# wljungbergh/mpc-trajectory-generator

Hardware: AMD Instinct MI355X
Metric: nmpc_solves_per_sec (higher is better)
Workload: dtype f64

## Files before the change

### mpc_trajectory_generator_amd/csrc/nmpc_eval.h

```cpp
#pragma once

namespace nmpc {

struct WinState {
    int ctr;
    double xr, yr, mo2;
};
struct ObsCert {
    double xo, yo, m2;
    int act_lo, act_hi, act_dyn;
};
__device__ __forceinline__ int opaque_i(int x) { asm("" : "+v"(x)); return x; }
__device__ __forceinline__ bool window_is_global(double a2, double best, double mo2)
{
    const double t = mo2 - (a2 + best);
    return t > 1e-5 * mo2 && t * t > 4.0001 * (a2 * best);
}

__device__ __forceinline__ unsigned long long circle_near_mask(const double *p, int N, int nobs, int lane, double radius)
{
    const double *ps = p + NZ + N;
    bool keep = false;
    if (lane < nobs) {
        const double dx = ps[3 * lane] - p[0], dy = ps[3 * lane + 1] - p[1], r = ps[3 * lane + 2], lim = radius + r;
        keep = r > 0.0 && fma(dx, dx, dy * dy) <= lim * lim;
    }
    return __ballot(keep);
}

struct EvK { double ts, inv_ts, amin, amax, awmax; };
__device__ __forceinline__ double scalar_own(double x)
{
    int lo = __double2loint(x), hi = __double2hiint(x);
    asm volatile("" : "+v"(lo), "+v"(hi));
    return __hiloint2double(__builtin_amdgcn_readfirstlane(hi), __builtin_amdgcn_readfirstlane(lo));
}
__device__ __forceinline__ int scalar_own(int x)
{
    asm volatile("" : "+v"(x));
    return __builtin_amdgcn_readfirstlane(x);
}
struct EvX {
    double vprev, wprev;
    lds_double2 *mine;
    const lds_double2 *next;
};
template <int P, class SH = ShapeAny, bool WRITE_F2 = false, bool CULL = false, int WIN = 0, bool Z60 = false>
__device__ __forceinline__ void eval_psi(const KArgs &a, lds_double *L, int f2off, int lane, int t, double zv, double zw,
                                         double c, double cbar_inv, double yv, double yw, double vref, const DynStage &dyn,
                                         bool want_grad, double &psi, double &pen_out, double &gv,
                                         double &gw, double &av_out, double &aw_out, unsigned long long near = ~0ull, WinState *ws = nullptr,
                                         ObsCert *oc = nullptr, long long *nmpc_pe = nullptr, const EvK *ek = nullptr, const EvX *evx = nullptr)
{
    static_assert(!Z60 || P == 20, "zero pads in lanes 60..63: the tri layout only");
    const int N = shape_N<SH>(a), nobs = shape_nobs<SH>(a), ndyn = shape_ndyn<SH>(a);
    const LdsMap mp = the_map<SH, P>(a);
    const double ts = ek ? ek->ts : a.pb.ts, inv_ts = ek ? ek->inv_ts : a.inv_ts;
    const double k_amin = ek ? ek->amin : a.pb.amin, k_amax = ek ? ek->amax : a.pb.amax, k_awmax = ek ? ek->awmax : a.pb.awmax;
    (void)nmpc_pe;
    constexpr bool FULL = P == 20 && SH::N == 20;
    const bool in_r = t < N;
    const bool in = FULL ? true : in_r;
    const lds_double *sc = L + mp.sc;
    const double x0 = sc[SC_X0], y0 = sc[SC_Y0], th0 = sc[SC_TH0];
    const double xf = sc[SC_XF], yf = sc[SC_YF], thf = sc[SC_THF];

    double ew_, ex_, ey_;
    auto prefix_ex = [lane](double v, double &excl) {
        if constexpr (Z60) return group_prefix_ex_z60(v, lane, excl);
        else return group_prefix_ex<P>(v, lane, excl);
    };
    const double thn = fma(ts, prefix_ex(zw, ew_), th0);
    const double th = t == 0 ? th0 : fma(ts, ew_, th0);
    double sn, cs;
    sincos_cw_t(th, (const lds_double *)(L + mp.cw), sn, cs);
    const double xn = fma(ts, prefix_ex(zv * cs, ex_), x0);
    const double yn = fma(ts, prefix_ex(zv * sn, ey_), y0);
    const double xp = t == 0 ? x0 : fma(ts, ex_, x0);
    const double yp = t == 0 ? y0 : fma(ts, ey_, y0);

    const double half_c = 0.5 * c;
    NMPC_EVTICK(nmpc_pe, 0);

    double acc = (sc[SC_RV] * zv) * zv;
    acc = fma(sc[SC_RW] * zw, zw, acc);
    const double dv = zv - vref;
    acc = fma(sc[SC_QV] * dv, dv, acc);
    {
        const double ddx = xp - xf, ddy = yp - yf, dth = th - thf;
        acc = fma(sc[SC_Q], fma(ddx, ddx, ddy * ddy), acc);
        acc = fma(sc[SC_QTH] * dth, dth, acc);
    }
    double best = __builtin_inf();
    int bi = 0;
    bool full_scan = true;
    int i0c = 0;
    if constexpr (WIN > 0) {
        const int nseg = N - 1;
        if (nseg >= 2 * WIN + 1) {
            int cc = ws->ctr;
            cc = cc < 0 ? 0 : (cc > nseg - 1 ? nseg - 1 : cc);
            i0c = cc - WIN;
            i0c = i0c < 0 ? 0 : (i0c > nseg - (2 * WIN + 1) ? nseg - (2 * WIN + 1) : i0c);
            if (!__any(in_r & !(ws->mo2 > 0.0))) {
                const lds_double *sg = L + mp.seg + SEG_STRIDE * i0c;
                double wv[2 * WIN + 1][5];
#pragma unroll
                for (int j = 0; j <= 2 * WIN; ++j)
#pragma unroll
                    for (int f = 0; f < 5; ++f) wv[j][f] = sg[j * SEG_STRIDE + f];
#pragma unroll
                for (int j = 0; j <= 2 * WIN; ++j) {
                    const double px = xn - wv[j][0], py = yn - wv[j][1];
                    const double dot = fma(px, wv[j][2], py * wv[j][3]);
                    const double that = dot * wv[j][4];
                    const double tst = fmin(fmax(that, 0.0), 1.0);
                    const double ex = fma(tst, wv[j][2], -px), ey = fma(tst, wv[j][3], -py);
                    const double d2 = fma(ex, ex, ey * ey);
                    bi = d2 < best ? i0c + j : bi;
                    best = fmin(best, d2);
                }
                const double ax = xn - ws->xr, ay = yn - ws->yr;
                const bool sure = window_is_global(fma(ax, ax, ay * ay), best, ws->mo2);
                full_scan = __any(in_r & !sure);
                NMPC_WIN_COUNT(0, full_scan);
                if (full_scan) {
                    i0c = bi - WIN;
                    i0c = i0c < 0 ? 0 : (i0c > nseg - (2 * WIN + 1) ? nseg - (2 * WIN + 1) : i0c);
                    best = __builtin_inf(); bi = 0;
                }
            }
        }
    }
    if (full_scan) {
        const lds_double *sg = L + mp.seg;
        const int nseg4 = (N - 1 + 3) & ~3;
        double cur[2][5], nxt[2][5];
        double mout = __builtin_inf();
#pragma unroll
        for (int j = 0; j < 2; ++j)
#pragma unroll
            for (int f = 0; f < 5; ++f) cur[j][f] = sg[j * SEG_STRIDE + f];
#pragma unroll SH::N > 0 ? (SH::N <= 20 ? 32 : 2) : 1
        for (int i = 0; i < nseg4; i += 2) {
            sg += 2 * SEG_STRIDE;
#pragma unroll
            for (int j = 0; j < 2; ++j)
#pragma unroll
                for (int f = 0; f < 5; ++f) nxt[j][f] = sg[j * SEG_STRIDE + f];
            NMPC_SCHED_BARRIER();
            double d2[2];
#pragma unroll
            for (int j = 0; j < 2; ++j) {
                const double px = xn - cur[j][0], py = yn - cur[j][1];
                const double dot = fma(px, cur[j][2], py * cur[j][3]);
                const double that = dot * cur[j][4];
                const double tst = fmin(fmax(that, 0.0), 1.0);
                const double ex = fma(tst, cur[j][2], -px), ey = fma(tst, cur[j][3], -py);
                d2[j] = fma(ex, ex, ey * ey);
            }
#pragma unroll
            for (int j = 0; j < 2; ++j) {
                bi = d2[j] < best ? i + j : bi;
                best = fmin(best, d2[j]);
                if constexpr (WIN > 0) {
                    const int ie = i + j < N - 1 ? i + j : N - 2;
                    mout = (unsigned)(ie - i0c) <= 2u * WIN ? mout : fmin(mout, d2[j]);
                }
            }
            NMPC_SCHED_BARRIER();
#pragma unroll
            for (int j = 0; j < 2; ++j)
#pragma unroll
                for (int f = 0; f < 5; ++f) cur[j][f] = nxt[j][f];
        }
        if constexpr (WIN > 0) {
            const bool inw = (unsigned)(bi - i0c) <= 2u * WIN;
            ws->ctr = inw ? i0c + WIN : bi;
            ws->xr = xn; ws->yr = yn;
            ws->mo2 = inw && mout > 1e-8 ? mout : 0.0;
        }
    }
    NMPC_EVTICK(nmpc_pe, 1);
    acc = fma(sc[SC_QCTE], best, acc);
    const double vprev = evx ? evx->vprev : from_prev<P>(zv, lane, sc[SC_VINIT]);
    const double wprev = evx ? evx->wprev : from_prev<P>(zw, lane, sc[SC_WINIT]);
    double av = (zv - vprev) * inv_ts, aw = (zw - wprev) * inv_ts;
    acc = fma(sc[SC_PA] * av, av, acc);
    acc = fma(sc[SC_PW] * aw, aw, acc);
    const double tv = fma(yv, cbar_inv, av), tw = fma(yw, cbar_inv, aw);
    double sv = tv - clampd(tv, k_amin, k_amax);
    double sw = tw - clampd(tw, -k_awmax, k_awmax);
    acc = fma(half_c, fma(sv, sv, sw * sw), acc);
    if (t == N - 1) {
        const double tx = xn - xf, ty = yn - yf, tth = thn - thf;
        acc = fma(sc[SC_QN], fma(tx, tx, ty * ty), acc);
        acc = fma(sc[SC_QTHN] * tth, tth, acc);
    }
    if (!in) { acc = 0.0; av = aw = sv = sw = 0.0; }
    av_out = av;
    aw_out = aw;
    const double fsum = group_sum<P>(acc, lane);
    NMPC_EVTICK(nmpc_pe, 2);

    double pen = 0.0;
    unsigned long long act = 0ull;
    unsigned act_dyn = 0u;
    bool scan = true;
    if (oc) {
        const double ox = xn - oc->xo, oy = yn - oc->yo;
        const bool sure = fma(ox, ox, oy * oy) < oc->m2;
        if (!__any(in_r & !sure)) {
            act = ((unsigned long long)(unsigned)__builtin_amdgcn_readfirstlane(oc->act_hi) << 32) | (unsigned)__builtin_amdgcn_readfirstlane(oc->act_lo);
            act_dyn = (unsigned)__builtin_amdgcn_readfirstlane(oc->act_dyn);
            scan = false;
        }
        NMPC_WIN_COUNT(2, scan);
    }
    if (scan) {
        double mg = __builtin_inf();
        const lds_double *ob = L + mp.obs;
        const int nobs4 = (nobs + 3) & ~3;
        if constexpr (CULL) {
            const unsigned long long all = nobs >= 64 ? ~0ull : (1ull << nobs) - 1ull;
            unsigned long long todo = near & all;
            if (todo != all) {
                const double rx = xn - x0, ry = yn - y0;
                const double rg = 0.999 * a.cull_radius;
                const double ro2 = fma(rx, rx, ry * ry);
                if (__any(in_r & !(ro2 <= rg * rg))) todo = all;
                else if (oc) mg = rg - __builtin_amdgcn_sqrt(ro2);
            }
            while (todo) {
                int kk[4];
#pragma unroll
                for (int j = 0; j < 4; ++j) {
                    kk[j] = todo ? __builtin_ctzll(todo) : nobs;
                    todo &= todo - (todo ? 1ull : 0ull);
                }
                double od[16];
#pragma unroll
                for (int j = 0; j < 4; ++j) {
                    const lds_double *oj = ob + OBS_STRIDE * kk[j];
                    od[4 * j] = oj[0]; od[4 * j + 1] = oj[1]; od[4 * j + 2] = oj[2]; od[4 * j + 3] = oc ? oj[3] : 0.0;
                }
                NMPC_SCHED_BARRIER();
#pragma unroll
                for (int j = 0; j < 4; ++j) {
                    const double dx = xn - od[4 * j], dy = yn - od[4 * j + 1];
                    const double h = fma(-dy, dy, fma(-dx, dx, od[4 * j + 2]));
                    if (__any(in_r & (h > 0.0))) act |= 1ull << (kk[j] & 63);
                    else if (oc) mg = fmin(mg, __builtin_amdgcn_sqrt(od[4 * j + 2] - h) - od[4 * j + 3]);
                }
            }
        } else {
#pragma unroll SH::NOBS >= 0 && SH::NOBS <= 16 ? 16 : 1
        for (int k = 0; k < nobs4; k += 4, ob += 4 * OBS_STRIDE) {
            double od[16];
#pragma unroll
            for (int j = 0; j < 4; ++j) {
                od[4 * j] = ob[OBS_STRIDE * j]; od[4 * j + 1] = ob[OBS_STRIDE * j + 1]; od[4 * j + 2] = ob[OBS_STRIDE * j + 2];
                od[4 * j + 3] = oc ? ob[OBS_STRIDE * j + 3] : 0.0;
            }
            NMPC_SCHED_BARRIER();
#pragma unroll
            for (int j = 0; j < 4; ++j) {
                const double dx = xn - od[4 * j], dy = yn - od[4 * j + 1];
                const double h = fma(-dy, dy, fma(-dx, dx, od[4 * j + 2]));
                if (__any(in_r & (h > 0.0))) act |= 1ull << (k + j);
                else if (oc) mg = fmin(mg, __builtin_amdgcn_sqrt(od[4 * j + 2] - h) - od[4 * j + 3]);
            }
        }
        }
        NMPC_EVTICK(nmpc_pe, 5);
        {
            double dv_[NDYN_MAX][DY_FIELDS];
#pragma unroll
            for (int k = 0; k < NDYN_MAX; ++k)
#pragma unroll
                for (int f = 0; f < DY_FIELDS; ++f) dv_[k][f] = k < ndyn ? dyn.get(k, f) : 0.0;
            NMPC_SCHED_BARRIER();
#pragma unroll
            for (int k = 0; k < NDYN_MAX; ++k) {
                if (k < ndyn) {
                    const double ca = dv_[k][DY_CA], sa = dv_[k][DY_SA];
                    const double dx = xn - dv_[k][DY_EX], dy = yn - dv_[k][DY_EY];
                    const double ea = fma(dx, ca, dy * sa);
                    const double eb = fma(dx, sa, -(dy * ca));
                    const double h = fma(-(eb * eb), dv_[k][DY_IRY2], fma(-(ea * ea), dv_[k][DY_IRX2], 1.0));
                    if (__any(in_r & (h > 0.0))) act_dyn |= 1u << k;
                    else if (oc)
                        mg = fmin(mg, __builtin_amdgcn_sqrt(fma(dx, dx, dy * dy)) - __builtin_amdgcn_rsq(fmin(dv_[k][DY_IRX2], dv_[k][DY_IRY2])));
                }
            }
        }
        if (oc) {
            const double m = fma(0.99, mg, -1e-6);
            oc->xo = xn; oc->yo = yn;
            oc->m2 = m > 0.0 ? (m < 1e100 ? m * m : 1e200) : 0.0;
            oc->act_lo = opaque_i((int)(unsigned)act); oc->act_hi = opaque_i((int)(unsigned)(act >> 32)); oc->act_dyn = opaque_i((int)act_dyn);
        }
        NMPC_EVTICK(nmpc_pe, 6);
    }
    double gx = 0.0, gy = 0.0;
    if (want_grad) {
        const lds_double *sg = L + mp.seg + SEG_STRIDE * bi;
        const double px = xn - sg[0], py = yn - sg[1];
        const double dot = fma(px, sg[2], py * sg[3]);
        const double that = dot * sg[4];
        const double tst = fmin(fmax(that, 0.0), 1.0);
        const double ex = fma(tst, sg[2], -px), ey = fma(tst, sg[3], -py);
        const double ed = fma(ex, sg[2], ey * sg[3]);
        const double m = (that > 0.0 && that < 1.0) ? ed * sg[4] : 0.0;
        const double two_q = 2.0 * sc[SC_QCTE];
        gx = two_q * fma(m, sg[2], -ex);
        gy = two_q * fma(m, sg[3], -ey);
    }
    if ((act | act_dyn) != 0ull) {
        for (unsigned long long rem = act; rem;) {
            const int k0 = __builtin_ctzll(rem);
            rem &= rem - 1;
            if (rem == 0ull) {
                const lds_double *o0 = L + mp.obs + OBS_STRIDE * k0;
                const double ax = o0[0], ay = o0[1], ar = o0[2];
                const double dx0 = xn - ax, dy0 = yn - ay;
                const double h0 = fma(-dy0, dy0, fma(-dx0, dx0, ar));
                const double f20 = group_sum<P>(in ? fmax(h0, 0.0) : 0.0, lane);
                if (WRITE_F2 && t == 0) L[f2off + k0] = f20;
                pen = fma(f20, f20, pen);
                if (want_grad) {
                    const double w0 = -2.0 * (c * f20);
                    if (h0 > 0.0) { gx = fma(w0, dx0, gx); gy = fma(w0, dy0, gy); }
                }
                break;
            }
            const int k1 = __builtin_ctzll(rem);
            rem &= rem - 1;
            const lds_double *o0 = L + mp.obs + OBS_STRIDE * k0, *o1 = L + mp.obs + OBS_STRIDE * k1;
            const double ax = o0[0], ay = o0[1], ar = o0[2], bx = o1[0], by = o1[1], br = o1[2];
            const double dx0 = xn - ax, dy0 = yn - ay, dx1 = xn - bx, dy1 = yn - by;
            const double h0 = fma(-dy0, dy0, fma(-dx0, dx0, ar)), h1 = fma(-dy1, dy1, fma(-dx1, dx1, br));
            const double f20 = group_sum<P>(in ? fmax(h0, 0.0) : 0.0, lane);
            const double f21 = group_sum<P>(in ? fmax(h1, 0.0) : 0.0, lane);
            if (WRITE_F2 && t == 0) { L[f2off + k0] = f20; L[f2off + k1] = f21; }
            pen = fma(f20, f20, pen);
            pen = fma(f21, f21, pen);
            if (want_grad) {
                const double w0 = -2.0 * (c * f20), w1 = -2.0 * (c * f21);
                if (h0 > 0.0) { gx = fma(w0, dx0, gx); gy = fma(w0, dy0, gy); }
                if (h1 > 0.0) { gx = fma(w1, dx1, gx); gy = fma(w1, dy1, gy); }
            }
        }
#pragma unroll
        for (int k = 0; k < NDYN_MAX; ++k) {
            if (act_dyn & (1u << k)) {
                const double ca = dyn.get(k, DY_CA), sa = dyn.get(k, DY_SA);
                const double irx2 = dyn.get(k, DY_IRX2), iry2 = dyn.get(k, DY_IRY2);
                const double dx = xn - dyn.get(k, DY_EX), dy = yn - dyn.get(k, DY_EY);
                const double ea = fma(dx, ca, dy * sa);
                const double eb = fma(dx, sa, -(dy * ca));
                const double h = fma(-(eb * eb), iry2, fma(-(ea * ea), irx2, 1.0));
                const double f2 = group_sum<P>(in ? fmax(h, 0.0) : 0.0, lane);
                if (WRITE_F2 && t == 0) L[f2off + nobs + k] = f2;
                pen = fma(f2, f2, pen);
                if (want_grad) {
                    const double wk = -2.0 * (c * f2);
                    if (h > 0.0) {
                        const double A = ea * irx2, Bq = eb * iry2;
                        const double hx = fma(A, ca, Bq * sa);
                        const double hy = fma(A, sa, -(Bq * ca));
                        gx = fma(wk, hx, gx);
                        gy = fma(wk, hy, gy);
                    }
                }
            }
        }
    }
    psi = fma(half_c, pen, fsum);
    pen_out = pen;
    NMPC_EVTICK(nmpc_pe, 3);
    if (!want_grad) return;

    const double wq = t < N - 1 ? sc[SC_Q] : sc[SC_QN];
    const double wth = t < N - 1 ? sc[SC_QTH] : sc[SC_QTHN];
    gx = fma(2.0 * wq, xn - xf, gx);
    gy = fma(2.0 * wq, yn - yf, gy);
    double gt = (2.0 * wth) * (thn - thf);
    double qa = fma(c, sv, (2.0 * sc[SC_PA]) * av);
    double qw = fma(c, sw, (2.0 * sc[SC_PW]) * aw);
    if (!in) { gx = gy = gt = qa = qw = 0.0; }
    const double Sx = group_suffix<P>(gx, lane);
    const double Sy = group_suffix<P>(gy, lane);
    const double e = fma(Sy, cs, -(Sx * sn));
    const double Dt = in ? (ts * zv) * e : 0.0;
    const double St = group_suffix<P>(in ? gt + from_next<P>(Dt, lane) : 0.0, lane);
    double qan, qwn;
    if (evx) { *evx->mine = dbl2{qa, qw}; const dbl2 n_ = *evx->next; qan = n_.x; qwn = n_.y; }
    else { qan = from_next<P>(qa, lane); qwn = from_next<P>(qw, lane); }
    const double dynv = fma(Sx, cs, Sy * sn);
    double g1 = fma(2.0 * sc[SC_RV], zv, (2.0 * sc[SC_QV]) * dv);
    g1 = fma(inv_ts, qa - qan, g1);
    g1 = fma(ts, dynv, g1);
    double g2 = (2.0 * sc[SC_RW]) * zw;
    g2 = fma(inv_ts, qw - qwn, g2);
    g2 = fma(ts, St, g2);
    gv = in ? g1 : 0.0;
    gw = in ? g2 : 0.0;
    NMPC_EVTICK(nmpc_pe, 4);
}

template <int P>
__device__ __forceinline__ double hdot(double av, double aw, double bv, double bw, int lane)
{
    return group_sum<P>(fma(av, bv, aw * bw), lane);
}

template <int P>
__global__ __launch_bounds__(64) void nmpc_eval_kernel(KArgs a)
{
    extern __shared__ double lds[];
    constexpr int K = 64 / P;
    const int lane = threadIdx.x, g = lay_group<P>(lane), t = lay_stage<P>(lane);
    lds_double *L = (lds_double *)lds + g * a.map.total;
    const int N = a.pb.N;
    const bool in = t < N;
    const int inst = blockIdx.x * K + g;
    const int b = inst < a.B ? inst : a.B - 1;
    double vref;
    DynStage dyn;
    prepare_instance<P>(a, L, a.p + (size_t)b * a.n_p, t, vref, dyn);
    const double *u = a.u + (size_t)b * a.n_u;
    const double zv = in ? u[2 * t] : 0.0, zw = in ? u[2 * t + 1] : 0.0;
    const double c = a.ev_c ? a.ev_c[b] : 0.0;
    const double yv = (a.ev_y && in) ? a.ev_y[(size_t)b * a.n1 + t] : 0.0;
    const double yw = (a.ev_y && in) ? a.ev_y[(size_t)b * a.n1 + N + t] : 0.0;
    for (int k = t; k < a.n2; k += P) L[a.map.f2 + k] = 0.0;
    NMPC_WAVE_SYNC();
    double psi, pen, gv, gw, av, aw;
    eval_psi<P, ShapeAny, true>(a, L, a.map.f2, lane, t, zv, zw, c, 1.0 / fmax(c, 1.0), yv, yw, vref, dyn, true, psi, pen, gv, gw, av, aw);
    NMPC_WAVE_SYNC();
    if (inst >= a.B) return;
    if (t == 0 && a.ev_psi) a.ev_psi[b] = psi;
    if (in) {
        if (a.ev_grad) { a.ev_grad[(size_t)b * a.n_u + 2 * t] = gv; a.ev_grad[(size_t)b * a.n_u + 2 * t + 1] = gw; }
        if (a.ev_F1) { a.ev_F1[(size_t)b * a.n1 + t] = av; a.ev_F1[(size_t)b * a.n1 + N + t] = aw; }
    }
    if (a.ev_F2) for (int k = t; k < a.n2; k += P) a.ev_F2[(size_t)b * a.n2 + k] = L[a.map.f2 + k];
}

}
```

### mpc_trajectory_generator_amd/csrc/nmpc_layout.h

```cpp
#pragma once

#ifndef NMPC_WIN
#define NMPC_WIN 1
#endif

namespace nmpc {

constexpr int NZ = 20;
constexpr int MAXMEM = 10;
constexpr int NDYN_MAX = 3;
constexpr int GRAM_LD = 11;
constexpr int GRAM_NST = 20;
constexpr int OBS_STRIDE = 4;
constexpr int SEG_STRIDE = 5;
constexpr int TEAM_WAVES = 4;
constexpr int TEAM_REQ_DOUBLES = 3 * 24 * 2;
constexpr int TEAM_AREA_DOUBLES = 3 * 24 * 2 + 8;
constexpr int TEAM_CTL_INTS = 64;
constexpr int NPOOLS = 2;
enum { POOL_LONG = 0, POOL_COLD = 1 };

constexpr double GAMMA_L_COEFF = 0.95;
constexpr double DELTA_LIPSCHITZ = 1e-12;
constexpr double EPSILON_LIPSCHITZ = 1e-6;
constexpr double LIPSCHITZ_UPDATE_EPSILON = 1e-6;
constexpr int MAX_LIPSCHITZ_UPDATE_ITERATIONS = 10;
constexpr double MAX_LIPSCHITZ_CONSTANT = 1e9;
constexpr double MIN_LIPSCHITZ_CONSTANT = 1e-10;
constexpr int MAX_LINESEARCH_ITERATIONS = 10;
constexpr double LBFGS_SY_EPSILON = 1e-10;
constexpr double LBFGS_CBFGS_EPSILON = 1e-8;

struct LdsMap {
    int sc;
    int cw;
    int par;
    int seg;
    int obs;
    int f2;
    int dyn;
    int dyn_stride;
    int req;
    int vec;
    int rho;
    int S, Y;
    int nv;
    int gsy, gyy;
    int total;
};

struct KArgs {
    nmpc_problem pb;
    nmpc_opts op;
    LdsMap map;
    int B;
    int n_p, n_u, n1, n2;
    double inv_ts;
    const double *p;
    double *u;
    const double *y0;
    const double *c0;
    double *y_out;
    nmpc_status *st;
    unsigned int *queue;
    const int *order;
    int park_min;
    int park_depth;
    double *park;
    int *pool;
    unsigned int *pool_ctr;
    int pool_cap;
    int sched_mode;
    int sched_long_cap;
    int sched_cold_cap;
    int dbg;
    int team_owners;
    int team_help;
    double cull_radius;
    union {
        struct {
            const double *ev_c;
            const double *ev_y;
            double *ev_psi, *ev_grad, *ev_F1, *ev_F2;
        };
        struct {
            long long tl_dur;
            long long tl_budget;
            const long long *tl_t0;
        };
    };
};

enum { SC_X0 = 0, SC_Y0, SC_TH0, SC_VINIT, SC_WINIT, SC_XF, SC_YF, SC_THF,
       SC_Q, SC_QV, SC_QTH, SC_RV, SC_RW, SC_QN, SC_QTHN, SC_QCTE, SC_PA, SC_PW };

typedef __attribute__((address_space(3))) double lds_double;
typedef double dbl2 __attribute__((ext_vector_type(2)));
typedef __attribute__((address_space(3))) dbl2 lds_double2;

#ifdef NMPC_NO_SCHED_BARRIER
#define NMPC_SCHED_BARRIER() do { } while (0)
#else
#define NMPC_SCHED_BARRIER() __builtin_amdgcn_sched_barrier(0)
#endif
#define NMPC_WAVE_SYNC()                                           \
    do {                                                           \
        __builtin_amdgcn_fence(__ATOMIC_RELEASE, "workgroup");     \
        __builtin_amdgcn_wave_barrier();                           \
        __builtin_amdgcn_fence(__ATOMIC_ACQUIRE, "workgroup");     \
    } while (0)

enum { DY_EX = 0, DY_EY, DY_CA, DY_SA, DY_IRX2, DY_IRY2, DY_FIELDS };
struct DynStage {
    const lds_double *col;
    int stride;
    __device__ __forceinline__ double get(int k, int f) const { return col[(k * DY_FIELDS + f) * stride]; }
};

struct ShapeAny { static constexpr int N = 0, NOBS = -1, NDYN = -1; };
struct ShapeDefault { static constexpr int N = 20, NOBS = 10, NDYN = 3; };
struct ShapeNobs50 { static constexpr int N = 20, NOBS = 50, NDYN = 3; };
struct ShapeN40 { static constexpr int N = 40, NOBS = 10, NDYN = 3; };
template <class S> struct Timed { static constexpr int N = S::N, NOBS = S::NOBS, NDYN = S::NDYN; };
template <class SH> struct ShapeTimed { static constexpr bool value = false; };
template <class S> struct ShapeTimed<Timed<S>> { static constexpr bool value = true; };
template <class SH> __device__ __forceinline__ int shape_N(const KArgs &a) { if constexpr (SH::N > 0) return SH::N; else return a.pb.N; }
template <class SH> __device__ __forceinline__ int shape_nobs(const KArgs &a) { if constexpr (SH::NOBS >= 0) return SH::NOBS; else return a.pb.nobs; }
template <class SH> __device__ __forceinline__ int shape_ndyn(const KArgs &a) { if constexpr (SH::NDYN >= 0) return SH::NDYN; else return a.pb.ndyn; }

__host__ __device__ constexpr LdsMap lds_layout(int N, int nobs, int ndyn, int P)
{
    LdsMap mp{};
    int o = 0;
    mp.sc = o;  o += 20;
    mp.cw = o;  o += CW_NCOEF;
    mp.par = o; o += 24;
    mp.seg = o; o += SEG_STRIDE * (N + 5);
    mp.obs = o; o += OBS_STRIDE * (nobs + 4);
    const int points = P == 64 ? 1 : 3;
    mp.f2 = o;  o += P == 20 ? 0 : points * (nobs + ndyn + 1);
    mp.rho = o; o += MAXMEM;
    const int cols = P == 20 ? 24 : P;
    mp.dyn_stride = P == 64 ? ((N + 1) & ~1) : (P == 20 ? 24 : P);
    mp.dyn = o; o += NDYN_MAX * 6 * mp.dyn_stride;
    o = (o + 1) & ~1;
    mp.req = o; o += P == 20 ? TEAM_REQ_DOUBLES : 0;
    mp.vec = o; o += P == 64 ? 0 : 7 * 2 * cols;
    if (P == 20) { mp.f2 = mp.vec; if (7 * 2 * cols < points * (nobs + ndyn + 1)) o = mp.vec + points * (nobs + ndyn + 1); }
    o = (o + 1) & ~1;
    mp.gsy = o; o += P == 20 ? MAXMEM * GRAM_LD : 0;
    mp.gyy = o; o += P == 20 ? MAXMEM * GRAM_LD : 0;
    const int ring = P == 20 ? GRAM_NST + 1 : N;
    mp.S = o;   o += 2 * ring * MAXMEM;
    mp.Y = o;   o += 2 * ring * MAXMEM;
    mp.nv = o;  o += P == 20 ? 4 * 2 * GRAM_NST : 0;
    mp.total = (o + 1) & ~1;
    if (P == 20 && mp.total < 3 * TEAM_WAVES * TEAM_AREA_DOUBLES) mp.total = 3 * TEAM_WAVES * TEAM_AREA_DOUBLES;
    return mp;
}
template <class SH, int P> __device__ __forceinline__ LdsMap the_map(const KArgs &a)
{
    if constexpr (SH::N > 0 && SH::NOBS >= 0 && SH::NDYN >= 0) return lds_layout(SH::N, SH::NOBS, SH::NDYN, P);
    else return a.map;
}

template <int P, class SH = ShapeAny>
__device__ __forceinline__ void prepare_instance(const KArgs &a, lds_double *L, const double *p, int t,
                                                 double &vref, DynStage &dyn)
{
    const int N = shape_N<SH>(a), nobs = shape_nobs<SH>(a), ndyn = shape_ndyn<SH>(a);
    const LdsMap mp = the_map<SH, P>(a);
    if (t < 8) L[mp.sc + t] = p[t];
    if (t >= 8 && t < 18) L[mp.sc + t] = p[t + 2];
    if (t == 18 || t == 19) L[mp.sc + t] = p[t - 15];
    if (t < CW_NCOEF) L[mp.cw + t] = CW_COEF_DEV[t];
    NMPC_WAVE_SYNC();
    vref = t < N ? p[NZ + t] : 0.0;
    const double *ps = p + NZ + N;
    for (int k = t; k < ((nobs + 4) & ~3); k += P) {
        const bool real = k < nobs;
        const double r = real ? ps[3 * k + 2] : 0.0;
        L[mp.obs + OBS_STRIDE * k] = real ? ps[3 * k] : 0.0;
        L[mp.obs + OBS_STRIDE * k + 1] = real ? ps[3 * k + 1] : 0.0;
        L[mp.obs + OBS_STRIDE * k + 2] = r * r;
        L[mp.obs + OBS_STRIDE * k + 3] = r > 0.0 ? r : -1e30;
    }
    const double *pd = ps + 3 * nobs;
    {
        lds_double *col = L + mp.dyn + t;
        dyn.col = col;
        const int ds = P == 64 ? mp.dyn_stride : lay_cols<P>();
        dyn.stride = ds;
#pragma unroll
        for (int k = 0; k < NDYN_MAX; ++k) {
            double ex = 0.0, ey = 0.0, ca = 0.0, sa = 0.0, irx2 = 1.0, iry2 = 1.0;
            if (k < ndyn && t < N) {
                const double *e = pd + (k * N + t) * 5;
                ex = e[0];
                ey = e[1];
                irx2 = 1.0 / (e[2] * e[2]);
                iry2 = 1.0 / (e[3] * e[3]);
                sincos_cw_t(e[4], (const lds_double *)(L + mp.cw), sa, ca);
            }
            if (P != 64 || t < ds) {
                col[(k * DY_FIELDS + DY_EX) * ds] = ex;
                col[(k * DY_FIELDS + DY_EY) * ds] = ey;
                col[(k * DY_FIELDS + DY_CA) * ds] = ca;
                col[(k * DY_FIELDS + DY_SA) * ds] = sa;
                col[(k * DY_FIELDS + DY_IRX2) * ds] = irx2;
                col[(k * DY_FIELDS + DY_IRY2) * ds] = iry2;
            }
        }
    }
    const double *pr = pd + 5 * ndyn * N;
    const int nseg4 = (N - 1 + 3) & ~3;
    if (t < nseg4) {
        const int i = t < N - 1 ? t : N - 2;
        const double ax = pr[3 * i], ay = pr[3 * i + 1];
        const double bx = pr[3 * i + 3], by = pr[3 * i + 4];
        const double dx = bx - ax, dy = by - ay;
        lds_double *sg = L + mp.seg + SEG_STRIDE * t;
        sg[0] = ax;
        sg[1] = ay;
        sg[2] = dx;
        sg[3] = dy;
        sg[4] = 1.0 / (fma(dx, dx, dy * dy) + 1e-16);
    }
    NMPC_WAVE_SYNC();
}

__host__ __device__ inline int park_stride(int N) { return 6 * N + 16; }
}
```

### mpc_trajectory_generator_amd/csrc/nmpc_solve_hyb.h

```cpp
#pragma once

#ifndef NMPC_CULL_MIN
#define NMPC_CULL_MIN 16
#endif
#ifndef NMPC_WIN
#define NMPC_WIN 1
#endif

namespace nmpc {

typedef __attribute__((address_space(3))) int lds_int;
enum { CTL_OWNERS = 0, CTL_HELPERS = 1, CTL_CLAIM = 4, CTL_DONE = 8, CTL_INST = 56 };
__device__ __forceinline__ int ctl_load(lds_int *p) { return __hip_atomic_load(p, __ATOMIC_RELAXED, __HIP_MEMORY_SCOPE_WORKGROUP); }
__device__ __forceinline__ void ctl_store(lds_int *p, int v) { __hip_atomic_store(p, v, __ATOMIC_RELAXED, __HIP_MEMORY_SCOPE_WORKGROUP); }
__device__ __forceinline__ int ctl_add(lds_int *p, int v) { return __hip_atomic_fetch_add(p, v, __ATOMIC_RELAXED, __HIP_MEMORY_SCOPE_WORKGROUP); }

__device__ __forceinline__ double point_scalar(double v, int k)
{
    const int lo = __builtin_amdgcn_readlane(__double2loint(v), 16 * k);
    const int hi = __builtin_amdgcn_readlane(__double2hiint(v), 16 * k);
    return __hiloint2double(hi, lo);
}

#define NMPC_FETCH_GRAD(K, OV, OW)                                             \
    do {                                                                       \
        const dbl2 fg_ = zgr[(K) * ZS];                                        \
        OV = fg_.x; OW = fg_.y;                                                \
    } while (0)

#define NMPC_HALF_STEP(xv, xw)                                                 \
    do {                                                                       \
        const double s1_ = fma(-gamma, gv, (xv)), s2_ = fma(-gamma, gw, (xw)); \
        hv = ina ? clampd(s1_, vmin, vmax) : s1_;                              \
        hw = ina ? clampd(s2_, -wmax, wmax) : s2_;                             \
    } while (0)
#define NMPC_FBE(xv, xw) fbe_value<P>(cost, gamma, pk_hig, fma(-gamma, gv, (xv)), fma(-gamma, gw, (xw)), hv, hw, gv, gw, lane)

constexpr int POOL_CTRS = 4;
__device__ __forceinline__ int pool_pop(const KArgs &a, int c)
{
    unsigned int *ctr = a.pool_ctr + POOL_CTRS * c;
    int *cnt = (int *)(ctr + 2);
    if (__hip_atomic_load(cnt, __ATOMIC_RELAXED, __HIP_MEMORY_SCOPE_AGENT) <= 0) return -1;
    if (__hip_atomic_fetch_add(cnt, -1, __ATOMIC_RELAXED, __HIP_MEMORY_SCOPE_AGENT) <= 0) {
        __hip_atomic_fetch_add(cnt, 1, __ATOMIC_RELAXED, __HIP_MEMORY_SCOPE_AGENT);
        return -1;
    }
    const unsigned pos = __hip_atomic_fetch_add(&ctr[0], 1u, __ATOMIC_RELAXED, __HIP_MEMORY_SCOPE_AGENT);
    int *slot = a.pool + (size_t)c * a.pool_cap + pos % (unsigned)a.pool_cap;
    int inst;
    do { inst = __hip_atomic_load(slot, __ATOMIC_ACQUIRE, __HIP_MEMORY_SCOPE_AGENT); } while (inst < 0);
    __hip_atomic_store(slot, -1, __ATOMIC_RELAXED, __HIP_MEMORY_SCOPE_AGENT);
    return inst;
}
__device__ __forceinline__ void pool_push(const KArgs &a, int c, int inst)
{
    unsigned int *ctr = a.pool_ctr + POOL_CTRS * c;
    const unsigned pos = __hip_atomic_fetch_add(&ctr[1], 1u, __ATOMIC_RELAXED, __HIP_MEMORY_SCOPE_AGENT);
    int *slot = a.pool + (size_t)c * a.pool_cap + pos % (unsigned)a.pool_cap;
    while (__hip_atomic_load(slot, __ATOMIC_RELAXED, __HIP_MEMORY_SCOPE_AGENT) >= 0) __builtin_amdgcn_s_sleep(1);
    __hip_atomic_store(slot, inst, __ATOMIC_RELEASE, __HIP_MEMORY_SCOPE_AGENT);
    __hip_atomic_fetch_add((int *)(ctr + 2), 1, __ATOMIC_RELEASE, __HIP_MEMORY_SCOPE_AGENT);
}
__device__ __forceinline__ int pool_depth(const KArgs &a, int c)
{
    return __hip_atomic_load((int *)(a.pool_ctr + POOL_CTRS * c + 2), __ATOMIC_RELAXED, __HIP_MEMORY_SCOPE_AGENT);
}

template <int J>
__device__ __forceinline__ double fnma_row_bcast(double acc, double x, double y)
{
    asm("s_nop 1\n\tv_fmac_f64_dpp %0, -%1, %2 row_newbcast:%3 row_mask:0xf bank_mask:0xf" : "+v"(acc) : "v"(x), "v"(y), "n"(J));
    return acc;
}
template <int J>
__device__ __forceinline__ double fma_row_bcast(double acc, double x, double y)
{
    asm("s_nop 1\n\tv_fmac_f64_dpp %0, %1, %2 row_newbcast:%3 row_mask:0xf bank_mask:0xf" : "+v"(acc) : "v"(x), "v"(y), "n"(J));
    return acc;
}
template <int J>
__device__ __forceinline__ void fnma3_row_bcast(double &a1, double &a2, double &a3, double x, double y1, double y2, double y3, double after)
{
    asm("v_fmac_f64_dpp %0, -%3, %4 row_newbcast:%8 row_mask:0xf bank_mask:0xf\n\t"
        "v_fmac_f64_dpp %1, -%3, %5 row_newbcast:%8 row_mask:0xf bank_mask:0xf\n\t"
        "v_fmac_f64_dpp %2, -%3, %6 row_newbcast:%8 row_mask:0xf bank_mask:0xf"
        : "+v"(a1), "+v"(a2), "+v"(a3) : "v"(x), "v"(y1), "v"(y2), "v"(y3), "v"(after), "n"(J));
}
template <int J>
__device__ __forceinline__ void fma2_row_bcast(double &a1, double &a2, double x, double y1, double y2, double after)
{
    asm("v_fmac_f64_dpp %0, %2, %3 row_newbcast:%6 row_mask:0xf bank_mask:0xf\n\t"
        "v_fmac_f64_dpp %1, %2, %4 row_newbcast:%6 row_mask:0xf bank_mask:0xf"
        : "+v"(a1), "+v"(a2) : "v"(x), "v"(y1), "v"(y2), "v"(after), "n"(J));
}
template <int J>
__device__ __forceinline__ void fnma2_row_bcast(double &a1, double &a2, double x, double y1, double y2, double after)
{
    asm("v_fmac_f64_dpp %0, -%2, %3 row_newbcast:%6 row_mask:0xf bank_mask:0xf\n\t"
        "v_fmac_f64_dpp %1, -%2, %4 row_newbcast:%6 row_mask:0xf bank_mask:0xf"
        : "+v"(a1), "+v"(a2) : "v"(x), "v"(y1), "v"(y2), "v"(after), "n"(J));
}
template <int J>
__device__ __forceinline__ void fnma5_row_bcast(double &a1, double &a2, double &a3, double &a4, double &a5, double x, double y1, double y2, double y3,
                                                double y4, double y5, double after)
{
    asm("v_fmac_f64_dpp %0, -%5, %6 row_newbcast:%12 row_mask:0xf bank_mask:0xf\n\t"
        "v_fmac_f64_dpp %1, -%5, %7 row_newbcast:%12 row_mask:0xf bank_mask:0xf\n\t"
        "v_fmac_f64_dpp %2, -%5, %8 row_newbcast:%12 row_mask:0xf bank_mask:0xf\n\t"
        "v_fmac_f64_dpp %3, -%5, %9 row_newbcast:%12 row_mask:0xf bank_mask:0xf\n\t"
        "v_fmac_f64_dpp %4, -%5, %10 row_newbcast:%12 row_mask:0xf bank_mask:0xf"
        : "+v"(a1), "+v"(a2), "+v"(a3), "+v"(a4), "+v"(a5) : "v"(x), "v"(y1), "v"(y2), "v"(y3), "v"(y4), "v"(y5), "v"(after), "n"(J));
}
template <int J>
__device__ __forceinline__ void fma4_row_bcast(double &a1, double &a2, double &a3, double &a4, double x, double y1, double y2, double y3, double y4,
                                               double after)
{
    asm("v_fmac_f64_dpp %0, %4, %5 row_newbcast:%10 row_mask:0xf bank_mask:0xf\n\t"
        "v_fmac_f64_dpp %1, %4, %6 row_newbcast:%10 row_mask:0xf bank_mask:0xf\n\t"
        "v_fmac_f64_dpp %2, %4, %7 row_newbcast:%10 row_mask:0xf bank_mask:0xf\n\t"
        "v_fmac_f64_dpp %3, %4, %8 row_newbcast:%10 row_mask:0xf bank_mask:0xf"
        : "+v"(a1), "+v"(a2), "+v"(a3), "+v"(a4) : "v"(x), "v"(y1), "v"(y2), "v"(y3), "v"(y4), "v"(after), "n"(J));
}
__device__ __forceinline__ double lane_scalar(double v, int ln)
{
    const int lo = __builtin_amdgcn_readlane(__double2loint(v), ln);
    const int hi = __builtin_amdgcn_readlane(__double2hiint(v), ln);
    return __hiloint2double(hi, lo);
}
template <int J>
__device__ __forceinline__ double gram_fwd_step(double &ga1, double &ga2, double &dv, double &dw, double rho, double gs, double gy, double alp,
                                                double ypx, double ypy)
{
    double al;
    asm("v_mul_f64 %0, %5, %1\n\t"
        "v_fmac_f64_dpp %3, -%8, %9 row_newbcast:%12 row_mask:0xf bank_mask:0xf\n\t"
        "v_fmac_f64_dpp %4, -%8, %10 row_newbcast:%12 row_mask:0xf bank_mask:0xf\n\t"
        "v_fmac_f64_dpp %1, -%0, %6 row_newbcast:%11 row_mask:0xf bank_mask:0xf\n\t"
        "v_fmac_f64_dpp %2, -%0, %7 row_newbcast:%11 row_mask:0xf bank_mask:0xf"
        : "=&v"(al), "+v"(ga1), "+v"(ga2), "+v"(dv), "+v"(dw)
        : "v"(rho), "v"(gs), "v"(gy), "v"(alp), "v"(ypx), "v"(ypy), "n"(J), "n"(J - 1));
    return al;
}
__device__ __forceinline__ double gram_fwd_first(double &ga1, double &ga2, double rho, double gs, double gy)
{
    double al;
    asm("v_mul_f64 %0, %3, %1\n\t"
        "s_nop 1\n\t"
        "v_fmac_f64_dpp %1, -%0, %4 row_newbcast:0 row_mask:0xf bank_mask:0xf\n\t"
        "v_fmac_f64_dpp %2, -%0, %5 row_newbcast:0 row_mask:0xf bank_mask:0xf"
        : "=&v"(al), "+v"(ga1), "+v"(ga2) : "v"(rho), "v"(gs), "v"(gy));
    return al;
}
template <int J>
__device__ __forceinline__ double gram_bwd_step(double &ga2, double &dv, double &dw, double rho, double alv, double gr, double abp, double spx,
                                                double spy)
{
    double ab;
    asm("v_mul_f64 %0, %4, %1\n\t"
        "v_add_f64 %0, %5, -%0\n\t"
        "v_fmac_f64_dpp %2, %7, %8 row_newbcast:%11 row_mask:0xf bank_mask:0xf\n\t"
        "v_fmac_f64_dpp %3, %7, %9 row_newbcast:%11 row_mask:0xf bank_mask:0xf\n\t"
        "v_fmac_f64_dpp %1, %0, %6 row_newbcast:%10 row_mask:0xf bank_mask:0xf"
        : "=&v"(ab), "+v"(ga2), "+v"(dv), "+v"(dw)
        : "v"(rho), "v"(alv), "v"(gr), "v"(abp), "v"(spx), "v"(spy), "n"(J), "n"(J + 1));
    return ab;
}
#define NMPC_GRAM_LDF(H, J)                                                                    \
        constexpr int fp##J = ((H) + (J)) % MAXMEM;                                            \
        const double fgs##J = Lgsy[pkrow + fp##J], fgy##J = Lgyy[pkrow + fp##J];               \
        const dbl2 fyp##J = LY[fp##J * NS + tt]
#define NMPC_GRAM_FWD(H, J, JP)                                                                \
        NMPC_GRAM_LDF(H, J);                                                                   \
        const double fal##J = gram_fwd_step<(J)>(ga1, ga2, dv, dw, rho_k, fgs##J, fgy##J, fal##JP, fyp##JP.x, fyp##JP.y)
#define NMPC_GRAM_LDB(H, J)                                                                    \
        constexpr int bp##J = ((H) + (J)) % MAXMEM;                                            \
        const double bgr##J = Lgsy[bp##J * GRAM_LD + pk_];                                     \
        const dbl2 bsp##J = LS[bp##J * NS + tt]
#define NMPC_GRAM_BWD(H, J, JP)                                                                \
        NMPC_GRAM_LDB(H, J);                                                                   \
        const double bab##J = gram_bwd_step<(J)>(ga2, dv, dw, rho_k, alv, bgr##J, bab##JP, bsp##JP.x, bsp##JP.y)
#define NMPC_GRAM_BOTH(H)                                                                                                            \
    do {                                                                                                                             \
        NMPC_GRAM_LDF(H, 0);                                                                                                         \
        const double fal0 = gram_fwd_first(ga1, ga2, rho_k, fgs0, fgy0);                                                             \
        NMPC_GRAM_FWD(H, 1, 0); NMPC_GRAM_FWD(H, 2, 1); NMPC_GRAM_FWD(H, 3, 2); NMPC_GRAM_FWD(H, 4, 3); NMPC_GRAM_FWD(H, 5, 4);      \
        NMPC_GRAM_FWD(H, 6, 5); NMPC_GRAM_FWD(H, 7, 6); NMPC_GRAM_FWD(H, 8, 7); NMPC_GRAM_FWD(H, 9, 8);                              \
        fnma2_row_bcast<9>(dv, dw, fal9, fyp9.x, fyp9.y, ga1);                                                                      \
        const double alv = rho_k * ga1;                        \
        ga2 = n_H0 * ga2;                                                                                                            \
        dv = n_H0 * dv; dw = n_H0 * dw;                                                                                              \
        NMPC_GRAM_LDB(H, 9);                                                                                                         \
        const double bab9 = alv - rho_k * ga2;                                                                                       \
        ga2 = fma_row_bcast<9>(ga2, bab9, bgr9);                                                                                     \
        NMPC_GRAM_BWD(H, 8, 9); NMPC_GRAM_BWD(H, 7, 8); NMPC_GRAM_BWD(H, 6, 7); NMPC_GRAM_BWD(H, 5, 6); NMPC_GRAM_BWD(H, 4, 5);      \
        NMPC_GRAM_BWD(H, 3, 4); NMPC_GRAM_BWD(H, 2, 3); NMPC_GRAM_BWD(H, 1, 2); NMPC_GRAM_BWD(H, 0, 1);                              \
        fma2_row_bcast<0>(dv, dw, bab0, bsp0.x, bsp0.y, ga2);                                                                        \
    } while (0)

struct FlagBit {
    unsigned &w;
    const unsigned bit;
    __device__ __forceinline__ operator bool() const { return (w & bit) != 0u; }
    __device__ __forceinline__ FlagBit &operator=(bool v) { w = v ? (w | bit) : (w & ~bit); return *this; }
    __device__ __forceinline__ FlagBit &operator=(const FlagBit &o) { return *this = (bool)o; }
};

template <class SH>
__global__ __launch_bounds__(64 * TEAM_WAVES, 2) void nmpc_solve_hyb_kernel(KArgs a)
{
    static_assert(MAXMEM == 10, "the Gram-form recurrences are written out for ten pairs");
    constexpr int PE = 20;
    constexpr int P = 32, COLS = 24;
    extern __shared__ double lds[];
    const int wid = __builtin_amdgcn_readfirstlane((int)(threadIdx.x >> 6));
    const int slice = the_map<SH, PE>(a).total;
    lds_double *L = (lds_double *)lds + wid * slice;
    lds_int *ctl = (lds_int *)((lds_double *)lds + TEAM_WAVES * slice);
    const int lane = threadIdx.x & 63, h = lane >> 5, t = lane & 31;
    const int q = lay_group<PE>(lane), te = lay_stage<PE>(lane);
    const int N = shape_N<SH>(a), m = scalar_own(a.op.lbfgs_memory);
    const int k_akkt = scalar_own(a.op.akkt_gradient), k_lsf = scalar_own(a.op.ls_failure);
#ifdef NMPC_EXPERIMENTS
    const int k_help = scalar_own(a.team_help), k_dbg = scalar_own(a.dbg);
#else
    constexpr int k_help = 1, k_dbg = 0;
#endif
    const bool in = t < N, ina = in;
    const bool ine = te < N;
    constexpr bool FULL = SH::N == PE;
    constexpr bool CULL = SH::NOBS > NMPC_CULL_MIN || SH::NOBS < 0;
    constexpr int WIN = NMPC_WIN;
    constexpr bool OBSC = SH::N > 0;
    const bool inea = FULL ? true : ine;
    const LdsMap mp = the_map<SH, PE>(a);
    const int n2 = shape_nobs<SH>(a) + shape_ndyn<SH>(a);
    const int f2off = mp.f2 + q * (n2 + 1);
    constexpr int ZS = 24, src0 = 0, src1 = 1, src2 = 2;
    static_assert(3 * ZS + 8 == 4 * GRAM_NST, "the transport area is the place of the Gram batch's four vectors");
    lds_double2 *Lz = (lds_double2 *)(L + mp.nv);
    lds_double2 *zwX = Lz + (t < ZS ? h * ZS + t : 3 * ZS + (t - ZS));
    lds_double2 *zwY = Lz + (t < ZS ? 2 * ZS + t : 3 * ZS + (t - ZS));
    const lds_double2 *zrd = Lz + q * ZS + te;
    const lds_double2 *zpv = te == 0 ? (const lds_double2 *)(L + mp.sc + 18) : (lane < 60 ? zrd - 1 : zrd);
    lds_double2 *zmine = Lz + (lane < 60 ? q * ZS + te : 3 * ZS + (lane - 60));
    const lds_double2 *znext = Lz + opaque_i(lane < 60 ? q * ZS + te + 1 : 3 * ZS + (lane - 60) + 1);
    const lds_double2 *zgr = Lz + (t < 20 ? t : 20);
    constexpr int NS = GRAM_NST + 1;
    const int tt = t < GRAM_NST ? t : GRAM_NST;
    lds_double2 *LS = (lds_double2 *)(L + mp.S);
    lds_double2 *LY = (lds_double2 *)(L + mp.Y);
    lds_double *Lrho = L + mp.rho;
    lds_double2 *Lnv = (lds_double2 *)(L + mp.nv);
    lds_double *Lgsy = L + mp.gsy, *Lgyy = L + mp.gyy;
    const int c16 = lane & 15, q4 = lane >> 4;
    lds_double2 *Los = (lds_double2 *)(L + mp.vec) + (t < COLS ? t : COLS - 1);
    lds_double2 *Log = Los + COLS, *Lq = Los + 2 * COLS, *Lyp = Los + 3 * COLS;
    lds_double2 *Lgk = Los + 6 * COLS;
    lds_double2 *LypE = (lds_double2 *)(L + mp.vec) + 3 * COLS + te;
    lds_double2 *Ly = (lds_double2 *)(L + mp.vec) + 4 * COLS + te;
    lds_double *Lvr = L + mp.vec + 2 * 5 * COLS + te;
#define NMPC_LB_ZERO()                                                                                  \
    do {                                                                                                \
        lds_double2 *z_ = (lds_double2 *)(L + mp.gsy);                                                  \
        for (int i_ = lane; i_ < MAXMEM * GRAM_LD + 2 * MAXMEM * NS; i_ += 64) z_[i_] = dbl2{0.0, 0.0};  \
        if (lane < MAXMEM) Lrho[lane] = 0.0;                                                            \
    } while (0)
    if (threadIdx.x < TEAM_CTL_INTS) ctl[threadIdx.x] = threadIdx.x == CTL_OWNERS ? a.team_owners : 0;
    __syncthreads();
    lds_double2 *Lreq = (lds_double2 *)(L + mp.req);
    unsigned team_seq = 0;
    const double vmin = scalar_own(a.pb.vmin), vmax = scalar_own(a.pb.vmax), wmax = scalar_own(a.pb.wmax);
    const EvK ek = {scalar_own(a.pb.ts), scalar_own(a.inv_ts), scalar_own(a.pb.amin), scalar_own(a.pb.amax), scalar_own(a.pb.awmax)};
    const double tol_ = scalar_own(a.op.tolerance);
    const unsigned max_inner = (unsigned)scalar_own(a.op.max_inner);
    const unsigned budget = (unsigned)scalar_own(a.op.max_total_inner);
    constexpr bool TIMED = ShapeTimed<SH>::value;
    long long clk_batch = CLK_NEVER, clk_dl = CLK_NEVER;
    if constexpr (TIMED) { if (a.tl_budget > 0) clk_batch = uniform_ll(*a.tl_t0) + a.tl_budget; }
    lds_double *Lpar = L + mp.par;
#define pk_eps_nu Lpar[0]
#define pk_dy_norm Lpar[1]
#define pk_f2_norm Lpar[2]
#define pk_dy_norm_plus Lpar[3]
#define pk_f2_norm_plus Lpar[4]
#define pk_last_fpr Lpar[5]
#define pk_last_cost Lpar[6]
#define pk_norm_h Lpar[7]
#define pk_Lc Lpar[8]
#define pk_H0 Lpar[9]
#define pk_sigma Lpar[10]
#define pk_c_lip Lpar[11]
#define pk_fbe_u Lpar[20]
#define pk_hig Lpar[19]
#define pk_gr Lpar[12]


    const unsigned hw_slot = __builtin_amdgcn_s_getreg(((4 - 1) << 11) | (0 << 6) | 4);
    const bool unfavoured = hw_slot != 0u;
    const int PS = park_stride(N);

    const int n_waves = (int)gridDim.x * TEAM_WAVES;
    if (a.order && unfavoured && a.park_min > 0 && a.B >= n_waves + (n_waves >> 2)) {
        const unsigned want = (unsigned)n_waves / 2;
        const long long t_hold = (long long)__builtin_amdgcn_s_memrealtime();
        while (__hip_atomic_load(a.queue, __ATOMIC_RELAXED, __HIP_MEMORY_SCOPE_AGENT) < want &&
               (long long)__builtin_amdgcn_s_memrealtime() - t_hold < 4000)
            __builtin_amdgcn_s_sleep(8);
    }

    for (; wid < a.team_owners;) {
        int fetched = -1, from_pool = 0;
        if (lane == 0) {
            const bool pools = a.park_min > 0 || a.sched_mode > 0;
            if (pools && !unfavoured) { fetched = pool_pop(a, POOL_LONG); from_pool = fetched >= 0; }
            if (fetched < 0) {
                const unsigned nxt = atomicAdd(a.queue, 1u);
                if (nxt < (unsigned)a.B) fetched = a.order ? a.order[nxt] : (int)nxt;
                else if (pools) {
                    for (int c = 0; c < NPOOLS && fetched < 0; ++c) fetched = pool_pop(a, c);
                    from_pool = fetched >= 0;
                }
            }
        }
        const int inst = __builtin_amdgcn_readfirstlane(fetched);
        const bool resumed = __builtin_amdgcn_readfirstlane(from_pool) != 0;
        if (inst < 0) break;

        const long long dbg_t0 = __builtin_amdgcn_s_memtime();
        const auto clk0_ = __builtin_amdgcn_s_memrealtime();
        long long t_first = (long long)clk0_;
        Lpar[13] = (double)clk0_; Lpar[14] = 0.0;
        if (k_dbg == 1) { if (hw_slot & 1u) __builtin_amdgcn_s_setprio(0); else __builtin_amdgcn_s_setprio(3); }
        double vref_;
        DynStage dyn;
        if (lane == 0) ctl_store(ctl + CTL_INST + wid, -1);
        __builtin_amdgcn_fence(__ATOMIC_RELEASE, "workgroup");
        prepare_instance<PE, SH>(a, L, a.p + (size_t)inst * a.n_p, te, vref_, dyn);
        *Lvr = vref_;
        WinState ws = {te < N - 1 ? te : N - 2, 0.0, 0.0, 0.0};
        ObsCert oc = {0.0, 0.0, 0.0, 0, 0, 0};
        __builtin_amdgcn_fence(__ATOMIC_RELEASE, "workgroup");
        if (lane == 0) ctl_store(ctl + CTL_INST + wid, inst);
        unsigned long long near = ~0ull;
        if constexpr (CULL) {
            near = circle_near_mask(a.p + (size_t)inst * a.n_p, N, shape_nobs<SH>(a), lane, a.cull_radius);
            if (lane == 0) { Lpar[18] = __hiloint2double((int)(near >> 32), (int)near); }
        }

        const double *pk = a.park + (size_t)inst * PS;
        const double *u0 = resumed ? pk : a.u + (size_t)inst * a.n_u;
        double uv = in ? u0[2 * t] : 0.0, uw = in ? u0[2 * t + 1] : 0.0;
        {
            double yv0, yw0;
            if (resumed) {
                yv0 = ine ? pk[2 * N + 2 * te] : 0.0;
                yw0 = ine ? pk[2 * N + 2 * te + 1] : 0.0;
            } else {
                yv0 = (a.y0 && ine) ? a.y0[(size_t)inst * a.n1 + te] : 0.0;
                yw0 = (a.y0 && ine) ? a.y0[(size_t)inst * a.n1 + N + te] : 0.0;
            }
            *LypE = dbl2{yv0, yw0};
            *Ly = dbl2{yv0, yw0};
        }
        *Lq = (resumed && in) ? dbl2{pk[4 * N + 2 * t], pk[4 * N + 2 * t + 1]} : dbl2{0.0, 0.0};
        double gv = 0, gw = 0, hv = 0, hw = 0, rv = 0, rw = 0, dv = 0, dw = 0;
        unsigned fl = 0u;
        FlagBit need_grad{fl, 1u << 0}; need_grad = true;
        double cost = 0, gamma = 0, tau = 1, rhs_ls = 0;
        pk_fbe_u = 0.0; pk_hig = 0.0;
        pk_Lc = 0.0; pk_sigma = 0.0; pk_H0 = 1.0;
        FlagBit fbe_ok{fl, 1u << 1};
        int iteration = 0, lip_it = 0, ls_n = 0, lb_active = 0, lb_head = 0;
        FlagBit lb_first{fl, 1u << 2}; lb_first = true;
        int n_active = 0, n_head = 0;
        FlagBit n_first{fl, 1u << 3}, n_take_old{fl, 1u << 4}; n_first = true;
        double n_H0 = 1;
        unsigned num_iter = 0;
        const double c0 = a.c0 ? a.c0[inst] : 0.0;
        double pen_c = c0 > 0.0 ? c0 : a.op.initial_penalty;
        double cbar_inv = 1.0 / fmax(pen_c, 1.0);
        pk_c_lip = 0.0;
        pk_eps_nu = a.op.initial_tolerance;
        pk_dy_norm = 0.0; pk_f2_norm = 0.0; pk_dy_norm_plus = DBL_MAX; pk_f2_norm_plus = 0.0; pk_last_fpr = 0.0; pk_last_cost = 0.0; pk_norm_h = 0.0;
        int nu = 0, inner_status = 0, state = D_INIT, final_status = 0;
        unsigned inner_total = 0, n_cost = 0, n_grad = 0, n_pass = 0;
        FlagBit parked{fl, 1u << 5};
        int park_cls = POOL_LONG;
        unsigned q_pass = 0;
        FlagBit long_counted{fl, 1u << 6};
        if (resumed) {
            const double *pks = a.park + (size_t)inst * PS + 6 * N;
            pen_c = pks[0];
            cbar_inv = 1.0 / fmax(pen_c, 1.0);
            pk_eps_nu = pks[1]; pk_dy_norm = pks[2]; pk_f2_norm = pks[3]; pk_dy_norm_plus = pks[4]; pk_f2_norm_plus = pks[5];
            pk_last_fpr = pks[6]; pk_last_cost = pks[7];
            nu = (int)pks[8]; inner_total = (unsigned)pks[9]; n_cost = (unsigned)pks[10]; n_grad = (unsigned)pks[11]; n_pass = (unsigned)pks[12];
            Lpar[13] = pks[13]; Lpar[14] = pks[14] + 1.0;
            if constexpr (TIMED) t_first = (long long)pks[13];
            long_counted = pks[15] != 0.0; q_pass = n_pass;
        }
        if constexpr (TIMED) clk_dl = clk_deadline(clk_batch, a.tl_dur, t_first);

        FlagBit f_start{fl, 1u << 7}, f_back{fl, 1u << 8}, f_trials{fl, 1u << 9}, f_begin{fl, 1u << 11}, f_done{fl, 1u << 12}, f_fb{fl, 1u << 13};
        FlagBit running{fl, 1u << 14}, timed_out{fl, 1u << 15};
        f_start = true; running = true;
        FlagBit posted{fl, 1u << 16};
        FlagBit clk_late{fl, 1u << 17};
        NMPC_PROBE_STATE

#define NMPC_END_ITERATION()                                                                                   \
        do {                                                                                                   \
            iteration++;                                                                                       \
            if (!(num_iter < max_inner)) f_done = true;                                                        \
            else {                                                                                             \
                num_iter++;                                                                                    \
                if ((budget > 0u && inner_total + num_iter >= budget) || (TIMED && clk_late)) { timed_out = true; f_done = true; } \
                else f_begin = true;                                                                           \
            }                                                                                                  \
        } while (0)
        for (;;) {
            double xv = 0, xw = 0, yqv = 0, yqw = 0;
            double nr2 = 0, norm_r = 0;
            double pv = 0, pw = 0;
            bool lb_batch = false;
            if (fl & (f_back.bit | f_fb.bit)) {
                if (f_back) {
                    if (posted) { posted = false; if (lane == 0) ctl_store(ctl + CTL_CLAIM + wid, 0); }
                    lb_active = 0; lb_first = true;
                    NMPC_LB_ZERO();
                    fbe_ok = false;
                    pk_Lc *= 2.0; gamma /= 2.0;
                    pk_sigma = (1.0 - GAMMA_L_COEFF) / (4.0 * gamma);
                    pk_c_lip = GAMMA_L_COEFF / (2.0 * gamma);
                    pk_hig = 0.5 / gamma;
                    NMPC_HALF_STEP(uv, uw);
                    lb_batch = true;
                }
                if (f_fb) {
                    f_fb = false;
                    tau = 0.0;
                    { const dbl2 gk_ = *Lgk; gv = gk_.x; gw = gk_.y; }
                    NMPC_HALF_STEP(uv, uw);
                    xv = yqv = hv; xw = yqw = hw; need_grad = true; state = D_FB;
                }
            }
            if (f_trials) {
                f_trials = false;
                const double th_ = h == 0 ? tau : tau / 2.0, omt = 1.0 - th_;
                xv = fma(-th_, dv, fma(-omt, rv, uv));
                xw = fma(-th_, dw, fma(-omt, rw, uw));
                const double t4_ = tau / 4.0, om4_ = 1.0 - t4_;
                yqv = fma(-t4_, dv, fma(-om4_, rv, uv));
                yqw = fma(-t4_, dw, fma(-om4_, rw, uw));
                need_grad = true; state = D_LS;
            }
            if (f_begin) lb_batch = true;
            if (f_begin) { NMPC_TL_STEP(); NMPC_TL_EV(tl_it, 0); }
            NMPC_SEC(0);
            double gU = 0.0, gs1 = 0.0, gs2 = 0.0, gy1 = 0.0, gy2 = 0.0;
            if (lb_batch) {
                rv = uv - hv; rw = uw - hw;
                if (f_begin && iteration >= 1 && !lb_first) {
                    const dbl2 os_ = *Los, og_ = *Log;
                    gs1 = uv - os_.x; gs2 = uw - os_.y; gy1 = rv - og_.x; gy2 = rw - og_.y;
                }
                if (t < GRAM_NST && h == 0) {
                    Lnv[t] = dbl2{gs1, gs2}; Lnv[GRAM_NST + t] = dbl2{gy1, gy2};
                    Lnv[2 * GRAM_NST + t] = dbl2{rv, rw}; Lnv[3 * GRAM_NST + t] = dbl2{gv, gw};
                }
                const lds_double2 *X1 = (c16 < MAXMEM ? LS + c16 * NS : (c16 == 11 ? Lnv + 2 * GRAM_NST : Lnv)) + 5 * q4;
                const lds_double2 *X2 = (c16 < MAXMEM ? LY + c16 * NS : (c16 == 11 ? Lnv + 3 * GRAM_NST : Lnv + GRAM_NST)) + 5 * q4;
                const lds_double2 *Z1 = (c16 < MAXMEM ? Lnv + GRAM_NST : (c16 == 10 ? Lnv : Lnv + 2 * GRAM_NST)) + 5 * q4;
                const lds_double2 *Z2 = (c16 < MAXMEM ? Lnv + 2 * GRAM_NST : (c16 == 10 ? Lnv + GRAM_NST : Lnv + 2 * GRAM_NST)) + 5 * q4;
                double V1 = 0.0, V2 = 0.0, V3 = 0.0, V4 = 0.0;
#pragma unroll
                for (int e = 0; e < 5; ++e) {
                    const dbl2 x1 = X1[e], x2 = X2[e], z1 = Z1[e], z2 = Z2[e];
                    V1 = fma(x1.x, z1.x, V1); V1 = fma(x1.y, z1.y, V1);
                    V2 = fma(x1.x, z2.x, V2); V2 = fma(x1.y, z2.y, V2);
                    V3 = fma(x2.x, z1.x, V3); V3 = fma(x2.y, z1.y, V3);
                    V4 = fma(x2.x, z2.x, V4); V4 = fma(x2.y, z2.y, V4);
                }
                swap_rows(V1, V2);
                const double W12 = V1 + V2;
                swap_rows(V3, V4);
                double W34 = V3 + V4;
                double W12b = W12;
                swap_halves(W12b, W34);
                gU = W12b + W34;
                nr2 = lane_scalar(gU, 11);
                pk_gr = lane_scalar(gU, 32 + 11);
                norm_r = sqrt(nr2);
                pk_last_fpr = norm_r;
                NMPC_SEC_KEEP(norm_r + gU);
            }
            NMPC_SEC(1);
            if (lb_batch) { NMPC_TL_KEEP(norm_r + gU); NMPC_TL_EV(tl_it, 1); }
            if (f_begin) {
                f_begin = false;
                bool exit_now = false;
                if (__any(norm_r < tol_)) {
                    if (k_akkt == 2) exit_now = true;
                    else if (k_akkt == 1 && iteration >= 1) {
                        exit_now = __any(norm_r < pk_eps_nu * gamma);
                    } else {
                        const dbl2 q_ = *Lq;
                        const bool top = k_akkt == 1;
                        const double b1 = top ? gv : gv - q_.x;
                        const double b2 = top ? gw : gw - q_.y;
                        const double a1 = rv / gamma + b1, a2 = rw / gamma + b2;
                        exit_now = __any(sqrt(group_sum<P>(fma(a1, a1, a2 * a2), lane)) < pk_eps_nu);
                    }
                }
                if (exit_now) {
                    f_done = true;
                } else if (iteration == 0) {
                    lip_it = 0;
                    xv = yqv = hv; xw = yqw = hw; need_grad = true; state = D_LIP;
                } else {
                    lip_it = 0;
                    n_first = lb_first; n_head = lb_head; n_active = lb_active; n_H0 = pk_H0; n_take_old = false;
                    bool took = false;
                    if (lb_first) {
                        n_first = false; n_take_old = true;
                    } else {
                        const double ss = lane_scalar(gU, 10), ys = lane_scalar(gU, 16 + 10);
                        bool ok = !(ss <= DBL_MIN || ys <= LBFGS_SY_EPSILON);
                        if (ok) ok = ys > (LBFGS_CBFGS_EPSILON * norm_r) * ss;
                        if (__any(ok)) {
                            took = true;
                            n_take_old = true;
                            n_head = lb_head == 0 ? MAXMEM - 1 : lb_head - 1;
                            if (in && h == 0) { LS[n_head * NS + t] = dbl2{gs1, gs2}; LY[n_head * NS + t] = dbl2{gy1, gy2}; }
                            if (lane == 0) Lrho[n_head] = 1.0 / ys;
                            const double yy = lane_scalar(gU, 48 + 10);
                            n_H0 = ys / yy;
                            if (n_active < m) n_active++;
                            if (c16 < MAXMEM && q4 < 3) {
                                const bool dg = c16 == n_head;
                                lds_double *wa = q4 == 0 ? Lgsy + c16 * GRAM_LD + n_head : (q4 == 1 ? Lgsy + n_head * GRAM_LD + c16 : Lgyy + c16 * GRAM_LD + n_head);
                                const double wv = q4 == 1 ? 0.0 : (dg ? (q4 == 0 ? 0.0 : yy) : gU);
                                *wa = wv;
                                if (q4 == 2) Lgyy[n_head * GRAM_LD + c16] = wv;
                            }
                            if (m < MAXMEM) {
                                const int ev = n_head + m >= MAXMEM ? n_head + m - MAXMEM : n_head + m;
// ... 492 lines not shown
```

### mpc_trajectory_generator_amd/csrc/nmpc_solve_hyb2.h

```cpp
#pragma once

namespace nmpc {

struct D2 { double a, b; };
__device__ __forceinline__ D2 d2s(double s) { return D2{s, s}; }
__device__ __forceinline__ D2 operator+(D2 x, D2 y) { return D2{x.a + y.a, x.b + y.b}; }
__device__ __forceinline__ D2 operator-(D2 x, D2 y) { return D2{x.a - y.a, x.b - y.b}; }
__device__ __forceinline__ D2 operator*(D2 x, D2 y) { return D2{x.a * y.a, x.b * y.b}; }
__device__ __forceinline__ D2 operator*(double s, D2 y) { return D2{s * y.a, s * y.b}; }
__device__ __forceinline__ D2 operator-(D2 x) { return D2{-x.a, -x.b}; }
__device__ __forceinline__ D2 fma2(D2 x, D2 y, D2 z) { return D2{fma(x.a, y.a, z.a), fma(x.b, y.b, z.b)}; }
__device__ __forceinline__ D2 fma2(double s, D2 y, D2 z) { return D2{fma(s, y.a, z.a), fma(s, y.b, z.b)}; }
__device__ __forceinline__ D2 fma2(double s, D2 y, double z) { return D2{fma(s, y.a, z), fma(s, y.b, z)}; }
__device__ __forceinline__ D2 sel2(bool ca, bool cb, D2 x, D2 y) { return D2{ca ? x.a : y.a, cb ? x.b : y.b}; }
__device__ __forceinline__ D2 clamp2(D2 x, double lo, double hi) { return D2{clampd(x.a, lo, hi), clampd(x.b, lo, hi)}; }

__device__ __forceinline__ double gsum2(D2 v, int lane) { return group_sum<20>(v.a + v.b, lane); }
__device__ __forceinline__ D2 gprefix2(D2 v, int lane)
{
    double E;
    const double W = group_prefix_ex<20>(v.a + v.b, lane, E);
    return D2{E + v.a, W};
}
__device__ __forceinline__ D2 gsuffix2(D2 v, int lane)
{
    const double Z = group_suffix<20>(v.a + v.b, lane);
    return D2{Z, from_next<20>(Z, lane) + v.b};
}
__device__ __forceinline__ D2 prev2(D2 v, int lane, double fill) { return D2{from_prev<20>(v.b, lane, fill), v.a}; }
__device__ __forceinline__ D2 next2(D2 v, int lane) { return D2{v.b, from_next<20>(v.a, lane)}; }

__device__ __forceinline__ double hdot2(D2 av, D2 aw, D2 bv, D2 bw) { return fma(av.a, bv.a, aw.a * bw.a) + fma(av.b, bv.b, aw.b * bw.b); }

template <int CNT> __device__ __forceinline__ void ld4(const lds_double2 *blk, int e, D2 &v, D2 &w)
{
    const dbl2 c0 = blk[e], c1 = blk[CNT + e];
    v = D2{c0.x, c1.x};
    w = D2{c0.y, c1.y};
}
template <int CNT> __device__ __forceinline__ void st4(lds_double2 *blk, int e, D2 v, D2 w)
{
    blk[e] = dbl2{v.a, w.a};
    blk[CNT + e] = dbl2{v.b, w.b};
}

struct LdsMap2 {
    int sc, cw, par, seg, obs, f2, rho;
    int dyn;
    int vr;
    int pts;
    int grd;
    int req;
    int vec;
    int gsy, gyy;
    int S, Y;
    int nv;
    int total;
};
#ifndef NMPC_WIN2
#define NMPC_WIN2 1
#endif
constexpr int H2_COLS = 24, H2_NS = 21, H2_ENT = 24;
constexpr int TEAM2_AREA_DOUBLES = 3 * H2_ENT * 4 + 8;
__host__ __device__ constexpr LdsMap2 lds_layout2(int N, int nobs, int ndyn)
{
    LdsMap2 mp{};
    int o = 0;
    mp.sc = o;  o += 20;
    mp.cw = o;  o += CW_NCOEF;
    mp.par = o; o += 20;
    mp.seg = o; o += SEG_STRIDE * (N + 5);
    mp.obs = o; o += OBS_STRIDE * (nobs + 4);
    mp.f2 = o;  o += 0;
    mp.rho = o; o += MAXMEM;
    o = (o + 1) & ~1;
    mp.dyn = o; o += NDYN_MAX * 6 * 48;
    mp.vr = o;  o += 48;
    mp.pts = o; o += 3 * H2_ENT * 4;
    mp.grd = o; o += 3 * H2_ENT * 4;
    mp.req = o; o += 3 * H2_ENT * 4;
    mp.vec = o; o += 7 * H2_COLS * 4;
    mp.f2 = mp.vec;
    if (7 * H2_COLS * 4 < 3 * (nobs + ndyn + 1)) o = mp.vec + 3 * (nobs + ndyn + 1);
    o = (o + 1) & ~1;
    mp.gsy = o; o += MAXMEM * GRAM_LD;
    mp.gyy = o; o += MAXMEM * GRAM_LD;
    mp.S = o;   o += MAXMEM * H2_NS * 4;
    mp.Y = o;   o += MAXMEM * H2_NS * 4;
    mp.nv = mp.pts;
    mp.total = (o + 1) & ~1;
    return mp;
}
template <class SH> __device__ __forceinline__ LdsMap2 the_map2(const KArgs &a)
{
    if constexpr (SH::N > 0 && SH::NOBS >= 0 && SH::NDYN >= 0) return lds_layout2(SH::N, SH::NOBS, SH::NDYN);
    else return lds_layout2(a.pb.N, a.pb.nobs, a.pb.ndyn);
}

template <class SH>
__device__ __forceinline__ void prepare_instance2(const KArgs &a, lds_double *L, const LdsMap2 &mp, const double *p, int lane)
{
    const int N = shape_N<SH>(a), nobs = shape_nobs<SH>(a), ndyn = shape_ndyn<SH>(a);
    if (lane < 8) L[mp.sc + lane] = p[lane];
    if (lane >= 8 && lane < 18) L[mp.sc + lane] = p[lane + 2];
    if (lane < CW_NCOEF) L[mp.cw + lane] = CW_COEF_DEV[lane];
    NMPC_WAVE_SYNC();
    if (lane < 48) L[mp.vr + lane] = lane < N ? p[NZ + lane] : 0.0;
    const double *ps = p + NZ + N;
    for (int k = lane; k < ((nobs + 3) & ~3); k += 64) {
        const bool real = k < nobs;
        const double r = real ? ps[3 * k + 2] : 0.0;
        L[mp.obs + OBS_STRIDE * k] = real ? ps[3 * k] : 0.0;
        L[mp.obs + OBS_STRIDE * k + 1] = real ? ps[3 * k + 1] : 0.0;
        L[mp.obs + OBS_STRIDE * k + 2] = r * r;
        L[mp.obs + OBS_STRIDE * k + 3] = r > 0.0 ? r : -1e30;
    }
    const double *pd = ps + 3 * nobs;
    if (lane < 48) {
        lds_double *col = L + mp.dyn + lane;
#pragma unroll
        for (int k = 0; k < NDYN_MAX; ++k) {
            double ex = 0.0, ey = 0.0, ca = 0.0, sa = 0.0, irx2 = 1.0, iry2 = 1.0;
            if (k < ndyn && lane < N) {
                const double *e = pd + (k * N + lane) * 5;
                ex = e[0];
                ey = e[1];
                irx2 = 1.0 / (e[2] * e[2]);
                iry2 = 1.0 / (e[3] * e[3]);
                sincos_cw_t(e[4], (const lds_double *)(L + mp.cw), sa, ca);
            }
            col[(k * DY_FIELDS + DY_EX) * 48] = ex;
            col[(k * DY_FIELDS + DY_EY) * 48] = ey;
            col[(k * DY_FIELDS + DY_CA) * 48] = ca;
            col[(k * DY_FIELDS + DY_SA) * 48] = sa;
            col[(k * DY_FIELDS + DY_IRX2) * 48] = irx2;
            col[(k * DY_FIELDS + DY_IRY2) * 48] = iry2;
        }
    }
    const double *pr = pd + 5 * ndyn * N;
    const int nseg4 = (N - 1 + 3) & ~3;
    if (lane < nseg4) {
        const int i = lane < N - 1 ? lane : N - 2;
        const double ax = pr[3 * i], ay = pr[3 * i + 1];
        const double bx = pr[3 * i + 3], by = pr[3 * i + 4];
        const double dx = bx - ax, dy = by - ay;
        lds_double *sg = L + mp.seg + SEG_STRIDE * lane;
        sg[0] = ax;
        sg[1] = ay;
        sg[2] = dx;
        sg[3] = dy;
        sg[4] = 1.0 / (fma(dx, dx, dy * dy) + 1e-16);
    }
    NMPC_WAVE_SYNC();
}

__device__ __forceinline__ D2 dyn2(const lds_double *L, const LdsMap2 &mp, int te, int k, int f)
{
    const dbl2 v = ((const lds_double2 *)(L + mp.dyn + (k * DY_FIELDS + f) * 48))[te];
    return D2{v.x, v.y};
}

struct ObsCert2 {
    D2 xo, yo, m2;
    int act_lo, act_hi, act_dyn;
};
template <class SH, bool WRITE_F2 = false, int WIN = 0>
__device__ __forceinline__ void eval_psi2(const KArgs &a, lds_double *L, const LdsMap2 &mp, int f2off, int lane, int te, D2 zv, D2 zw,
                                          double c, double cbar_inv, D2 yv, D2 yw, bool want_grad, double &psi, double &pen_out,
                                          D2 &gv, D2 &gw, D2 &av_out, D2 &aw_out, WinState *ws = nullptr, ObsCert2 *oc = nullptr)
{
    const int N = shape_N<SH>(a), nobs = shape_nobs<SH>(a), ndyn = shape_ndyn<SH>(a);
    const double ts = a.pb.ts, inv_ts = a.inv_ts;
    constexpr bool FULL = SH::N == 40;
    const int sa_ = 2 * te, sb_ = 2 * te + 1;
    const bool ra = sa_ < N, rb = sb_ < N;
    const bool ina = FULL ? true : ra, inb = FULL ? true : rb;
    const lds_double *sc = L + mp.sc;
    const lds_double *cw = (const lds_double *)(L + mp.cw);
    const double x0 = sc[SC_X0], y0 = sc[SC_Y0], th0 = sc[SC_TH0];
    const double xf = sc[SC_XF], yf = sc[SC_YF], thf = sc[SC_THF];
    D2 vref;
    { const dbl2 v = ((const lds_double2 *)(L + mp.vr))[te]; vref = D2{v.x, v.y}; }

    const D2 thn = fma2(ts, gprefix2(zw, lane), th0);
    const D2 th = prev2(thn, lane, th0);
    D2 sn, cs;
    sincos_cw_t(th.a, cw, sn.a, cs.a);
    sincos_cw_t(th.b, cw, sn.b, cs.b);
    const D2 xn = fma2(ts, gprefix2(zv * cs, lane), x0);
    const D2 yn = fma2(ts, gprefix2(zv * sn, lane), y0);
    const D2 xp = prev2(xn, lane, x0);
    const D2 yp = prev2(yn, lane, y0);
    const double half_c = 0.5 * c;

    D2 acc = (sc[SC_RV] * zv) * zv;
    acc = fma2(sc[SC_RW] * zw, zw, acc);
    const D2 dv = zv - vref;
    acc = fma2(sc[SC_QV] * dv, dv, acc);
    {
        const D2 ddx = xp - d2s(xf), ddy = yp - d2s(yf), dth = th - d2s(thf);
        acc = fma2(sc[SC_Q], fma2(ddx, ddx, ddy * ddy), acc);
        acc = fma2(sc[SC_QTH] * dth, dth, acc);
    }
    const D2 vprev = prev2(zv, lane, sc[SC_VINIT]);
    const D2 wprev = prev2(zw, lane, sc[SC_WINIT]);
    D2 best = d2s(__builtin_inf());
    int bia = 0, bib = 0;
    bool full_scan = true;
    int i0a = 0, i0b = 0;
    if constexpr (WIN > 0) {
        const int nseg = N - 1;
        if (nseg >= 2 * WIN + 1) {
#define NMPC2_CLAMP_WIN(C_) ((C_) - WIN < 0 ? 0 : ((C_) - WIN > nseg - (2 * WIN + 1) ? nseg - (2 * WIN + 1) : (C_) - WIN))
            { const int ca = ws[0].ctr < 0 ? 0 : (ws[0].ctr > nseg - 1 ? nseg - 1 : ws[0].ctr); i0a = NMPC2_CLAMP_WIN(ca); }
            { const int cb = ws[1].ctr < 0 ? 0 : (ws[1].ctr > nseg - 1 ? nseg - 1 : ws[1].ctr); i0b = NMPC2_CLAMP_WIN(cb); }
            if (!__any((ra & !(ws[0].mo2 > 0.0)) | (rb & !(ws[1].mo2 > 0.0)))) {
                bool sure_a, sure_b;
#define NMPC2_WINDOW(S_, BI_, I0_, WS_, SURE_)                                                             \
                do {                                                                                       \
                    const lds_double *sg = L + mp.seg + SEG_STRIDE * (I0_);                                \
                    double bst = __builtin_inf();                                                          \
                    int bi_ = 0;                                                                           \
                    _Pragma("unroll") for (int j = 0; j <= 2 * WIN; ++j) {                                 \
                        const double s0 = sg[j * SEG_STRIDE], s1 = sg[j * SEG_STRIDE + 1], s2 = sg[j * SEG_STRIDE + 2], \
                                     s3 = sg[j * SEG_STRIDE + 3], s4 = sg[j * SEG_STRIDE + 4];             \
                        const double px = xn.S_ - s0, py = yn.S_ - s1;                                     \
                        const double dot = fma(s2, px, s3 * py);                                           \
                        const double tst = fmin(fmax(s4 * dot, 0.0), 1.0);                                 \
                        const double ex = fma(s2, tst, -px), ey = fma(s3, tst, -py);                       \
                        const double d2 = fma(ex, ex, ey * ey);                                            \
                        bi_ = d2 < bst ? (I0_) + j : bi_;                                                  \
                        bst = fmin(bst, d2);                                                               \
                    }                                                                                      \
                    const double ax = xn.S_ - (WS_).xr, ay = yn.S_ - (WS_).yr;                             \
                    SURE_ = window_is_global(fma(ax, ax, ay * ay), bst, (WS_).mo2);                        \
                    best.S_ = bst; BI_ = bi_;                                                              \
                } while (0)
                NMPC2_WINDOW(a, bia, i0a, ws[0], sure_a);
                NMPC2_WINDOW(b, bib, i0b, ws[1], sure_b);
#undef NMPC2_WINDOW
                full_scan = __any((ra & !sure_a) | (rb & !sure_b));
                NMPC_WIN_COUNT(0, full_scan);
                if (full_scan) {
                    i0a = NMPC2_CLAMP_WIN(bia); i0b = NMPC2_CLAMP_WIN(bib);
                    best = d2s(__builtin_inf()); bia = bib = 0;
                }
            }
#undef NMPC2_CLAMP_WIN
        }
    }
    if (full_scan) {
        const lds_double *sg = L + mp.seg;
        const int nseg4 = (N - 1 + 3) & ~3;
        double cur[2][5], nxt[2][5];
        D2 mout = d2s(__builtin_inf());
#pragma unroll
        for (int j = 0; j < 2; ++j)
#pragma unroll
            for (int f = 0; f < 5; ++f) cur[j][f] = sg[j * SEG_STRIDE + f];
#pragma unroll SH::N > 0 ? 4 : 1
        for (int i = 0; i < nseg4; i += 2) {
            sg += 2 * SEG_STRIDE;
#pragma unroll
            for (int j = 0; j < 2; ++j)
#pragma unroll
                for (int f = 0; f < 5; ++f) nxt[j][f] = sg[j * SEG_STRIDE + f];
            NMPC_SCHED_BARRIER();
            D2 d2v[2];
#pragma unroll
            for (int j = 0; j < 2; ++j) {
                const D2 px = xn - d2s(cur[j][0]), py = yn - d2s(cur[j][1]);
                const D2 dot = fma2(cur[j][2], px, cur[j][3] * py);
                const D2 that = cur[j][4] * dot;
                const D2 tst = D2{fmin(fmax(that.a, 0.0), 1.0), fmin(fmax(that.b, 0.0), 1.0)};
                const D2 ex = fma2(cur[j][2], tst, -px), ey = fma2(cur[j][3], tst, -py);
                d2v[j] = fma2(ex, ex, ey * ey);
            }
#pragma unroll
            for (int j = 0; j < 2; ++j) {
                bia = d2v[j].a < best.a ? i + j : bia;
                bib = d2v[j].b < best.b ? i + j : bib;
                best = D2{fmin(best.a, d2v[j].a), fmin(best.b, d2v[j].b)};
                if constexpr (WIN > 0) {
                    const int ie = i + j < N - 1 ? i + j : N - 2;
                    mout.a = (unsigned)(ie - i0a) <= 2u * WIN ? mout.a : fmin(mout.a, d2v[j].a);
                    mout.b = (unsigned)(ie - i0b) <= 2u * WIN ? mout.b : fmin(mout.b, d2v[j].b);
                }
            }
            NMPC_SCHED_BARRIER();
#pragma unroll
            for (int j = 0; j < 2; ++j)
#pragma unroll
                for (int f = 0; f < 5; ++f) cur[j][f] = nxt[j][f];
        }
        if constexpr (WIN > 0) {
            const bool inwa = (unsigned)(bia - i0a) <= 2u * WIN, inwb = (unsigned)(bib - i0b) <= 2u * WIN;
            ws[0].ctr = inwa ? i0a + WIN : bia; ws[0].xr = xn.a; ws[0].yr = yn.a; ws[0].mo2 = inwa && mout.a > 1e-8 ? mout.a : 0.0;
            ws[1].ctr = inwb ? i0b + WIN : bib; ws[1].xr = xn.b; ws[1].yr = yn.b; ws[1].mo2 = inwb && mout.b > 1e-8 ? mout.b : 0.0;
        }
    }
    acc = fma2(sc[SC_QCTE], best, acc);
    D2 av = inv_ts * (zv - vprev), aw = inv_ts * (zw - wprev);
    acc = fma2(sc[SC_PA] * av, av, acc);
    acc = fma2(sc[SC_PW] * aw, aw, acc);
    const D2 tv = fma2(cbar_inv, yv, av), tw = fma2(cbar_inv, yw, aw);
    D2 sv = tv - clamp2(tv, a.pb.amin, a.pb.amax);
    D2 sw = tw - clamp2(tw, -a.pb.awmax, a.pb.awmax);
    acc = fma2(half_c, fma2(sv, sv, sw * sw), acc);
    if (sa_ == N - 1) {
        const double tx = xn.a - xf, ty = yn.a - yf, tth = thn.a - thf;
        acc.a = fma(sc[SC_QN], fma(tx, tx, ty * ty), acc.a);
        acc.a = fma(sc[SC_QTHN] * tth, tth, acc.a);
    }
    if (sb_ == N - 1) {
        const double tx = xn.b - xf, ty = yn.b - yf, tth = thn.b - thf;
        acc.b = fma(sc[SC_QN], fma(tx, tx, ty * ty), acc.b);
        acc.b = fma(sc[SC_QTHN] * tth, tth, acc.b);
    }
    if (!ina) { acc.a = 0.0; av.a = aw.a = sv.a = sw.a = 0.0; }
    if (!inb) { acc.b = 0.0; av.b = aw.b = sv.b = sw.b = 0.0; }
    av_out = av;
    aw_out = aw;
    const double fsum = gsum2(acc, lane);

    double pen = 0.0;
    unsigned long long act = 0ull;
    unsigned act_dyn = 0u;
    bool scan = true;
    if (oc) {
        const D2 ox = xn - oc->xo, oy = yn - oc->yo;
        const D2 o2 = fma2(ox, ox, oy * oy);
        if (!__any((ra & !(o2.a < oc->m2.a)) | (rb & !(o2.b < oc->m2.b)))) {
            act = ((unsigned long long)(unsigned)__builtin_amdgcn_readfirstlane(oc->act_hi) << 32) | (unsigned)__builtin_amdgcn_readfirstlane(oc->act_lo);
            act_dyn = (unsigned)__builtin_amdgcn_readfirstlane(oc->act_dyn);
            scan = false;
        }
        NMPC_WIN_COUNT(2, scan);
    }
    if (scan) {
        D2 mg = d2s(__builtin_inf());
        const lds_double *ob = L + mp.obs;
        const int nobs4 = (nobs + 3) & ~3;
#pragma unroll SH::NOBS >= 0 && SH::NOBS <= 16 ? 16 : 1
        for (int k = 0; k < nobs4; k += 4, ob += 4 * OBS_STRIDE) {
            double od[16];
#pragma unroll
            for (int j = 0; j < 4; ++j) {
                od[4 * j] = ob[OBS_STRIDE * j]; od[4 * j + 1] = ob[OBS_STRIDE * j + 1]; od[4 * j + 2] = ob[OBS_STRIDE * j + 2];
                od[4 * j + 3] = oc ? ob[OBS_STRIDE * j + 3] : 0.0;
            }
            NMPC_SCHED_BARRIER();
#pragma unroll
            for (int j = 0; j < 4; ++j) {
                if (SH::NOBS >= 0 && SH::NOBS <= 16 && k + j >= SH::NOBS) continue;
                const D2 dx = xn - d2s(od[4 * j]), dy = yn - d2s(od[4 * j + 1]);
                const D2 h = fma2(-dy, dy, fma2(-dx, dx, d2s(od[4 * j + 2])));
                if (__any((ra & (h.a > 0.0)) | (rb & (h.b > 0.0)))) act |= 1ull << (k + j);
                else if (oc) {
                    mg.a = fmin(mg.a, __builtin_amdgcn_sqrt(od[4 * j + 2] - h.a) - od[4 * j + 3]);
                    mg.b = fmin(mg.b, __builtin_amdgcn_sqrt(od[4 * j + 2] - h.b) - od[4 * j + 3]);
                }
            }
        }
#pragma unroll
        for (int k = 0; k < NDYN_MAX; ++k) {
            if (k < ndyn) {
                const D2 ca = dyn2(L, mp, te, k, DY_CA), sa = dyn2(L, mp, te, k, DY_SA);
                const D2 dx = xn - dyn2(L, mp, te, k, DY_EX), dy = yn - dyn2(L, mp, te, k, DY_EY);
                const D2 ea = fma2(dx, ca, dy * sa);
                const D2 eb = fma2(dx, sa, -(dy * ca));
                const D2 irx2 = dyn2(L, mp, te, k, DY_IRX2), iry2 = dyn2(L, mp, te, k, DY_IRY2);
                const D2 h = fma2(-(eb * eb), iry2, fma2(-(ea * ea), irx2, d2s(1.0)));
                if (__any((ra & (h.a > 0.0)) | (rb & (h.b > 0.0)))) act_dyn |= 1u << k;
                else if (oc) {
                    mg.a = fmin(mg.a, __builtin_amdgcn_sqrt(fma(dx.a, dx.a, dy.a * dy.a)) - __builtin_amdgcn_rsq(fmin(irx2.a, iry2.a)));
                    mg.b = fmin(mg.b, __builtin_amdgcn_sqrt(fma(dx.b, dx.b, dy.b * dy.b)) - __builtin_amdgcn_rsq(fmin(irx2.b, iry2.b)));
                }
            }
        }
        if (oc) {
            const D2 m = fma2(0.99, mg, -1e-6);
            oc->xo = xn; oc->yo = yn;
            oc->m2 = D2{m.a > 0.0 ? (m.a < 1e100 ? m.a * m.a : 1e200) : 0.0, m.b > 0.0 ? (m.b < 1e100 ? m.b * m.b : 1e200) : 0.0};
            oc->act_lo = opaque_i((int)(unsigned)act); oc->act_hi = opaque_i((int)(unsigned)(act >> 32)); oc->act_dyn = opaque_i((int)act_dyn);
        }
    }
    D2 gx = d2s(0.0), gy = d2s(0.0);
    if (want_grad) {
        const double two_q = 2.0 * sc[SC_QCTE];
#define NMPC_CTE_ADJ(S_, BI_)                                                              \
        do {                                                                               \
            const lds_double *sg = L + mp.seg + SEG_STRIDE * (BI_);                        \
            const double px = xn.S_ - sg[0], py = yn.S_ - sg[1];                           \
            const double dot = fma(px, sg[2], py * sg[3]);                                 \
            const double that = dot * sg[4];                                               \
            const double tst = fmin(fmax(that, 0.0), 1.0);                                 \
            const double ex = fma(tst, sg[2], -px), ey = fma(tst, sg[3], -py);             \
            const double ed = fma(ex, sg[2], ey * sg[3]);                                  \
            const double m = (that > 0.0 && that < 1.0) ? ed * sg[4] : 0.0;                \
            gx.S_ = two_q * fma(m, sg[2], -ex);                                            \
            gy.S_ = two_q * fma(m, sg[3], -ey);                                            \
        } while (0)
        NMPC_CTE_ADJ(a, bia);
        NMPC_CTE_ADJ(b, bib);
#undef NMPC_CTE_ADJ
    }
    if ((act | act_dyn) != 0ull) {
        for (unsigned long long rem = act; rem;) {
            const int k0 = __builtin_ctzll(rem);
            rem &= rem - 1;
            const lds_double *o0 = L + mp.obs + OBS_STRIDE * k0;
            const double ax = o0[0], ay = o0[1], ar = o0[2];
            const D2 dx0 = xn - d2s(ax), dy0 = yn - d2s(ay);
            const D2 h0 = fma2(-dy0, dy0, fma2(-dx0, dx0, d2s(ar)));
            const double f20 = gsum2(D2{ina ? fmax(h0.a, 0.0) : 0.0, inb ? fmax(h0.b, 0.0) : 0.0}, lane);
            if (WRITE_F2 && te == 0) L[f2off + k0] = f20;
            pen = fma(f20, f20, pen);
            if (want_grad) {
                const double w0 = -2.0 * (c * f20);
                if (h0.a > 0.0) { gx.a = fma(w0, dx0.a, gx.a); gy.a = fma(w0, dy0.a, gy.a); }
                if (h0.b > 0.0) { gx.b = fma(w0, dx0.b, gx.b); gy.b = fma(w0, dy0.b, gy.b); }
            }
        }
#pragma unroll
        for (int k = 0; k < NDYN_MAX; ++k) {
            if (act_dyn & (1u << k)) {
                const D2 ca = dyn2(L, mp, te, k, DY_CA), sa = dyn2(L, mp, te, k, DY_SA);
                const D2 irx2 = dyn2(L, mp, te, k, DY_IRX2), iry2 = dyn2(L, mp, te, k, DY_IRY2);
                const D2 dx = xn - dyn2(L, mp, te, k, DY_EX), dy = yn - dyn2(L, mp, te, k, DY_EY);
                const D2 ea = fma2(dx, ca, dy * sa);
                const D2 eb = fma2(dx, sa, -(dy * ca));
                const D2 h = fma2(-(eb * eb), iry2, fma2(-(ea * ea), irx2, d2s(1.0)));
                const double f2 = gsum2(D2{ina ? fmax(h.a, 0.0) : 0.0, inb ? fmax(h.b, 0.0) : 0.0}, lane);
                if (WRITE_F2 && te == 0) L[f2off + nobs + k] = f2;
                pen = fma(f2, f2, pen);
                if (want_grad) {
                    const double wk = -2.0 * (c * f2);
                    const D2 A = ea * irx2, Bq = eb * iry2;
                    const D2 hx = fma2(A, ca, Bq * sa);
                    const D2 hy = fma2(A, sa, -(Bq * ca));
                    if (h.a > 0.0) { gx.a = fma(wk, hx.a, gx.a); gy.a = fma(wk, hy.a, gy.a); }
                    if (h.b > 0.0) { gx.b = fma(wk, hx.b, gx.b); gy.b = fma(wk, hy.b, gy.b); }
                }
            }
        }
    }
    psi = fma(half_c, pen, fsum);
    pen_out = pen;
    if (!want_grad) return;

    const D2 wq = D2{sa_ < N - 1 ? sc[SC_Q] : sc[SC_QN], sb_ < N - 1 ? sc[SC_Q] : sc[SC_QN]};
    const D2 wth = D2{sa_ < N - 1 ? sc[SC_QTH] : sc[SC_QTHN], sb_ < N - 1 ? sc[SC_QTH] : sc[SC_QTHN]};
    gx = fma2(2.0 * wq, xn - d2s(xf), gx);
    gy = fma2(2.0 * wq, yn - d2s(yf), gy);
    D2 gt = (2.0 * wth) * (thn - d2s(thf));
    D2 qa = fma2(c, sv, (2.0 * sc[SC_PA]) * av);
    D2 qw = fma2(c, sw, (2.0 * sc[SC_PW]) * aw);
    if (!ina) { gx.a = gy.a = gt.a = qa.a = qw.a = 0.0; }
    if (!inb) { gx.b = gy.b = gt.b = qa.b = qw.b = 0.0; }
    const D2 Sx = gsuffix2(gx, lane);
    const D2 Sy = gsuffix2(gy, lane);
    const D2 e = fma2(Sy, cs, -(Sx * sn));
    D2 Dt = (ts * zv) * e;
    if (!ina) Dt.a = 0.0;
    if (!inb) Dt.b = 0.0;
    D2 stin = gt + next2(Dt, lane);
    if (!ina) stin.a = 0.0;
    if (!inb) stin.b = 0.0;
    const D2 St = gsuffix2(stin, lane);
    const D2 qan = next2(qa, lane), qwn = next2(qw, lane);
    const D2 dynv = fma2(Sx, cs, Sy * sn);
    D2 g1 = fma2(2.0 * sc[SC_RV], zv, (2.0 * sc[SC_QV]) * dv);
    g1 = fma2(inv_ts, qa - qan, g1);
    g1 = fma2(ts, dynv, g1);
    D2 g2 = (2.0 * sc[SC_RW]) * zw;
    g2 = fma2(inv_ts, qw - qwn, g2);
    g2 = fma2(ts, St, g2);
    gv = D2{ina ? g1.a : 0.0, inb ? g1.b : 0.0};
    gw = D2{ina ? g2.a : 0.0, inb ? g2.b : 0.0};
}

__global__ __launch_bounds__(64) void nmpc_eval2_kernel(KArgs a)
{
    extern __shared__ double lds[];
    const int lane = threadIdx.x, g = lay_group<20>(lane), te = lay_stage<20>(lane);
    const LdsMap2 mp = lds_layout2(a.pb.N, a.pb.nobs, a.pb.ndyn);
    const int N = a.pb.N;
    int b3[3];
#pragma unroll
    for (int k = 0; k < 3; ++k) {
        const int inst = blockIdx.x * 3 + k;
        b3[k] = inst < a.B ? inst : a.B - 1;
        lds_double *Lk = (lds_double *)lds + k * mp.total;
        prepare_instance2<ShapeAny>(a, Lk, mp, a.p + (size_t)b3[k] * a.n_p, lane);
        for (int j = lane; j < a.n2; j += 64) Lk[mp.f2 + j] = 0.0;
    }
    NMPC_WAVE_SYNC();
    lds_double *L = (lds_double *)lds + g * mp.total;
    const int inst = blockIdx.x * 3 + g;
    const int b = b3[0] * (g == 0) + b3[1] * (g == 1) + b3[2] * (g == 2);
    const bool ra = 2 * te < N, rb = 2 * te + 1 < N;
    const double *u = a.u + (size_t)b * a.n_u;
    const D2 zv = D2{ra ? u[4 * te] : 0.0, rb ? u[4 * te + 2] : 0.0}, zw = D2{ra ? u[4 * te + 1] : 0.0, rb ? u[4 * te + 3] : 0.0};
    const double c = a.ev_c ? a.ev_c[b] : 0.0;
    const double *yb = a.ev_y ? a.ev_y + (size_t)b * a.n1 : nullptr;
    const D2 yv = D2{(yb && ra) ? yb[2 * te] : 0.0, (yb && rb) ? yb[2 * te + 1] : 0.0};
    const D2 yw = D2{(yb && ra) ? yb[N + 2 * te] : 0.0, (yb && rb) ? yb[N + 2 * te + 1] : 0.0};
    double psi, pen;
    D2 gv, gw, av, aw;
    eval_psi2<ShapeAny, true>(a, L, mp, mp.f2, lane, te, zv, zw, c, 1.0 / fmax(c, 1.0), yv, yw, true, psi, pen, gv, gw, av, aw);
    NMPC_WAVE_SYNC();
    if (inst >= a.B) return;
    if (te == 0 && a.ev_psi) a.ev_psi[b] = psi;
    if (a.ev_grad) {
        double *go = a.ev_grad + (size_t)b * a.n_u;
        if (ra) { go[4 * te] = gv.a; go[4 * te + 1] = gw.a; }
        if (rb) { go[4 * te + 2] = gv.b; go[4 * te + 3] = gw.b; }
    }
    if (a.ev_F1) {
        double *fo = a.ev_F1 + (size_t)b * a.n1;
        if (ra) { fo[2 * te] = av.a; fo[N + 2 * te] = aw.a; }
        if (rb) { fo[2 * te + 1] = av.b; fo[N + 2 * te + 1] = aw.b; }
    }
    if (a.ev_F2 && te < 20) for (int k = te; k < a.n2; k += 20) a.ev_F2[(size_t)b * a.n2 + k] = L[mp.f2 + k];
}

template <int J>
__device__ __forceinline__ double gram2_fwd_step(double &ga1, double &ga2, double &dva, double &dvb, double &dwa, double &dwb, double rho, double gs,
                                                 double gy, double alp, double y1a, double y1b, double y2a, double y2b)
{
    double al;
    asm("v_mul_f64 %0, %7, %1\n\t"
        "v_fmac_f64_dpp %3, -%10, %11 row_newbcast:%16 row_mask:0xf bank_mask:0xf\n\t"
        "v_fmac_f64_dpp %4, -%10, %12 row_newbcast:%16 row_mask:0xf bank_mask:0xf\n\t"
        "v_fmac_f64_dpp %5, -%10, %13 row_newbcast:%16 row_mask:0xf bank_mask:0xf\n\t"
        "v_fmac_f64_dpp %6, -%10, %14 row_newbcast:%16 row_mask:0xf bank_mask:0xf\n\t"
        "v_fmac_f64_dpp %1, -%0, %8 row_newbcast:%15 row_mask:0xf bank_mask:0xf\n\t"
        "v_fmac_f64_dpp %2, -%0, %9 row_newbcast:%15 row_mask:0xf bank_mask:0xf"
        : "=&v"(al), "+v"(ga1), "+v"(ga2), "+v"(dva), "+v"(dvb), "+v"(dwa), "+v"(dwb)
        : "v"(rho), "v"(gs), "v"(gy), "v"(alp), "v"(y1a), "v"(y1b), "v"(y2a), "v"(y2b), "n"(J), "n"(J - 1));
    return al;
}
template <int J>
__device__ __forceinline__ double gram2_bwd_step(double &ga2, double &dva, double &dvb, double &dwa, double &dwb, double rho, double alv, double gr,
                                                 double abp, double s1a, double s1b, double s2a, double s2b)
{
    double ab;
    asm("v_mul_f64 %0, %6, %1\n\t"
        "v_add_f64 %0, %7, -%0\n\t"
        "v_fmac_f64_dpp %2, %9, %10 row_newbcast:%15 row_mask:0xf bank_mask:0xf\n\t"
        "v_fmac_f64_dpp %3, %9, %11 row_newbcast:%15 row_mask:0xf bank_mask:0xf\n\t"
        "v_fmac_f64_dpp %4, %9, %12 row_newbcast:%15 row_mask:0xf bank_mask:0xf\n\t"
        "v_fmac_f64_dpp %5, %9, %13 row_newbcast:%15 row_mask:0xf bank_mask:0xf\n\t"
        "v_fmac_f64_dpp %1, %0, %8 row_newbcast:%14 row_mask:0xf bank_mask:0xf"
        : "=&v"(ab), "+v"(ga2), "+v"(dva), "+v"(dvb), "+v"(dwa), "+v"(dwb)
        : "v"(rho), "v"(alv), "v"(gr), "v"(abp), "v"(s1a), "v"(s1b), "v"(s2a), "v"(s2b), "n"(J), "n"(J + 1));
    return ab;
}
template <int J>
__device__ __forceinline__ void fnma4_row_bcast(double &a1, double &a2, double &a3, double &a4, double x, double y1, double y2, double y3, double y4,
                                                double after)
{
    asm("v_fmac_f64_dpp %0, -%4, %5 row_newbcast:%10 row_mask:0xf bank_mask:0xf\n\t"
        "v_fmac_f64_dpp %1, -%4, %6 row_newbcast:%10 row_mask:0xf bank_mask:0xf\n\t"
        "v_fmac_f64_dpp %2, -%4, %7 row_newbcast:%10 row_mask:0xf bank_mask:0xf\n\t"
        "v_fmac_f64_dpp %3, -%4, %8 row_newbcast:%10 row_mask:0xf bank_mask:0xf"
        : "+v"(a1), "+v"(a2), "+v"(a3), "+v"(a4) : "v"(x), "v"(y1), "v"(y2), "v"(y3), "v"(y4), "v"(after), "n"(J));
}

__device__ __forceinline__ double fbe_value2(double cost, double gamma, double hig, D2 sv, D2 sw, D2 hv, D2 hw, D2 gv, D2 gw, int lane)
{
    const D2 e1 = sv - hv, e2 = sw - hw;
    double dist2, gg;
    pair_sum(hdot2(e1, e2, e1, e2), hdot2(gv, gw, gv, gw), lane, dist2, gg);
    return cost - (0.5 * gamma) * gg + dist2 * hig;
}

#define NMPC2_HALF_STEP(xv, xw)                                                                    \
    do {                                                                                           \
        const D2 s1_ = fma2(-gamma, gv, (xv)), s2_ = fma2(-gamma, gw, (xw));                       \
        hv = D2{ina ? clampd(s1_.a, vmin, vmax) : s1_.a, inb ? clampd(s1_.b, vmin, vmax) : s1_.b}; \
        hw = D2{ina ? clampd(s2_.a, -wmax, wmax) : s2_.a, inb ? clampd(s2_.b, -wmax, wmax) : s2_.b}; \
    } while (0)
#define NMPC2_FBE(xv, xw) fbe_value2(cost, gamma, Lpar[19], fma2(-gamma, gv, (xv)), fma2(-gamma, gw, (xw)), hv, hw, gv, gw, lane)
#define NMPC2_LOAD_GRAD(BASE, OV, OW)                                          \
    do {                                                                       \
        D2 fv_, fw_;                                                           \
        ld4<H2_ENT>((BASE), tz, fv_, fw_);                                        \
        OV = D2{ina ? fv_.a : 0.0, inb ? fv_.b : 0.0};                         \
        OW = D2{ina ? fw_.a : 0.0, inb ? fw_.b : 0.0};                         \
    } while (0)

template <class SH>
__global__ __launch_bounds__(64 * TEAM_WAVES, 1) void nmpc_solve_hyb2_kernel(KArgs a)
{
    constexpr int P = 32;
    extern __shared__ double lds[];
    const int wid = __builtin_amdgcn_readfirstlane((int)(threadIdx.x >> 6));
    const LdsMap2 mp = the_map2<SH>(a);
    const int slice = mp.total;
    lds_double *L = (lds_double *)lds + wid * slice;
    lds_int *ctl = (lds_int *)((lds_double *)lds + TEAM_WAVES * slice);
    const int lane = threadIdx.x & 63, h = lane >> 5, t = lane & 31;
    const int q = lay_group<20>(lane), te = lay_stage<20>(lane);
    const int N = shape_N<SH>(a), m = a.op.lbfgs_memory;
    const int NP = (N + 1) >> 1;
    const bool in = t < NP, ina = in, inb = 2 * t + 1 < N;
    constexpr bool FULL = SH::N == 40;
    const bool rea = 2 * te < N, reb = 2 * te + 1 < N;
    const bool inea = FULL ? true : rea, ineb = FULL ? true : reb;
    const int n2 = shape_nobs<SH>(a) + shape_ndyn<SH>(a);
    const int f2off = mp.f2 + q * (n2 + 1);
    const int tz = in ? t : 0, tt = t < H2_NS - 1 ? t : H2_NS - 1;
    const int tc = t < H2_COLS ? t : H2_COLS - 1;
    lds_double2 *Lnv = (lds_double2 *)(L + mp.nv);
    lds_double *Lgsy = L + mp.gsy, *Lgyy = L + mp.gyy;
    const int c16 = lane & 15, q4 = lane >> 4;
#define NMPC2_LB_ZERO()                                                                                    \
    do {                                                                                                   \
        lds_double2 *z_ = (lds_double2 *)(L + mp.gsy);                                                     \
        for (int i_ = lane; i_ < MAXMEM * GRAM_LD + 4 * MAXMEM * H2_NS; i_ += 64) z_[i_] = dbl2{0.0, 0.0};  \
        if (lane < MAXMEM) Lrho[lane] = 0.0;                                                               \
    } while (0)
    lds_double2 *LS = (lds_double2 *)(L + mp.S);
    lds_double2 *LY = (lds_double2 *)(L + mp.Y);
    lds_double *Lrho = L + mp.rho;
    lds_double2 *V = (lds_double2 *)(L + mp.vec);
    lds_double2 *Cos = V + 2 * H2_COLS * 0, *Cog = V + 2 * H2_COLS * 1, *Cq = V + 2 * H2_COLS * 2, *Cyp = V + 2 * H2_COLS * 3, *Cy = V + 2 * H2_COLS * 4,
                *Cgk = V + 2 * H2_COLS * 6;
    lds_double2 *Pts = (lds_double2 *)(L + mp.pts), *Grd = (lds_double2 *)(L + mp.grd), *Lreq = (lds_double2 *)(L + mp.req);
    if (threadIdx.x < TEAM_CTL_INTS) ctl[threadIdx.x] = threadIdx.x == CTL_OWNERS ? a.team_owners : 0;
    __syncthreads();
    unsigned team_seq = 0;
    const double vmin = a.pb.vmin, vmax = a.pb.vmax, wmax = a.pb.wmax;
    const unsigned max_inner = (unsigned)a.op.max_inner;
    const unsigned budget = (unsigned)a.op.max_total_inner;
    constexpr bool TIMED = ShapeTimed<SH>::value;
    long long clk_batch = CLK_NEVER, clk_dl = CLK_NEVER;
    if constexpr (TIMED) { if (a.tl_budget > 0) clk_batch = uniform_ll(*a.tl_t0) + a.tl_budget; }
    lds_double *Lpar = L + mp.par;

    for (; wid < a.team_owners;) {
        int fetched = -1, from_pool = 0;
        if (lane == 0) {
            const unsigned nxt = atomicAdd(a.queue, 1u);
            if (nxt < (unsigned)a.B) fetched = a.order ? a.order[nxt] : (int)nxt;
            else if (a.sched_mode > 0) {
                for (int c = 0; c < NPOOLS && fetched < 0; ++c) fetched = pool_pop(a, c);
                from_pool = fetched >= 0;
            }
        }
        const int inst = __builtin_amdgcn_readfirstlane(fetched);
        const bool resumed = __builtin_amdgcn_readfirstlane(from_pool) != 0;
        if (inst < 0) break;
        long long t_start = (long long)__builtin_amdgcn_s_memrealtime();
        if (lane == 0) ctl_store(ctl + CTL_INST + wid, -1);
        __builtin_amdgcn_fence(__ATOMIC_RELEASE, "workgroup");
        prepare_instance2<SH>(a, L, mp, a.p + (size_t)inst * a.n_p, lane);
        WinState ws[2] = {{2 * te < N - 1 ? 2 * te : N - 2, 0.0, 0.0, 0.0}, {2 * te + 1 < N - 1 ? 2 * te + 1 : N - 2, 0.0, 0.0, 0.0}};
        ObsCert2 oc = {d2s(0.0), d2s(0.0), d2s(0.0), 0, 0, 0};
        __builtin_amdgcn_fence(__ATOMIC_RELEASE, "workgroup");
        if (lane == 0) ctl_store(ctl + CTL_INST + wid, inst);

        const double *pk = a.park + (size_t)inst * park_stride(N);
        const double *u0 = resumed ? pk : a.u + (size_t)inst * a.n_u;
        D2 uv = D2{ina ? u0[4 * t] : 0.0, inb ? u0[4 * t + 2] : 0.0}, uw = D2{ina ? u0[4 * t + 1] : 0.0, inb ? u0[4 * t + 3] : 0.0};
        {
            const double *yb = resumed ? pk + 2 * N : (a.y0 ? a.y0 + (size_t)inst * a.n1 : nullptr);
            const D2 yv0 = D2{(yb && rea) ? yb[2 * te] : 0.0, (yb && reb) ? yb[2 * te + 1] : 0.0};
            const D2 yw0 = D2{(yb && rea) ? yb[N + 2 * te] : 0.0, (yb && reb) ? yb[N + 2 * te + 1] : 0.0};
            st4<H2_COLS>(Cyp, te, yv0, yw0);
            st4<H2_COLS>(Cy, te, yv0, yw0);
        }
        {
            const double *qb = pk + 4 * N;
            const bool ld = resumed && ina;
            st4<H2_COLS>(Cq, tc, D2{ld ? qb[4 * t] : 0.0, (ld && inb) ? qb[4 * t + 2] : 0.0}, D2{ld ? qb[4 * t + 1] : 0.0, (ld && inb) ? qb[4 * t + 3] : 0.0});
        }
        D2 gv = d2s(0.0), gw = d2s(0.0), hv = d2s(0.0), hw = d2s(0.0), rv = d2s(0.0), rw = d2s(0.0), dv = d2s(0.0), dw = d2s(0.0);
        D2 pv = d2s(0.0), pw = d2s(0.0);
        D2 xv = d2s(0.0), xw = d2s(0.0);
        D2 yqv = d2s(0.0), yqw = d2s(0.0);
        unsigned fl = 0u;
        FlagBit need_grad{fl, 1u << 0}; need_grad = true;
        double cost = 0, gamma = 0, nr2 = 0, norm_r = 0, tau = 1, rhs_ls = 0;
        double Lc = 0, sigma = 0, H0 = 1, c_lip = 0, gr = 0, norm_h = 0;
        double eps_nu = a.op.initial_tolerance, dy_norm = 0, f2_norm = 0, dy_norm_plus = DBL_MAX, f2_norm_plus = 0, last_fpr = 0, last_cost = 0;
        double fbe_u = 0;
        FlagBit fbe_ok{fl, 1u << 1};
        int iteration = 0, lip_it = 0, ls_n = 0, lb_active = 0, lb_head = 0;
        FlagBit lb_first{fl, 1u << 2}; lb_first = true;
        int n_active = 0, n_head = 0;
        FlagBit n_first{fl, 1u << 3}, n_take_old{fl, 1u << 4}; n_first = true;
        double n_H0 = 1;
        unsigned num_iter = 0;
        const double c0 = a.c0 ? a.c0[inst] : 0.0;
        double pen_c = c0 > 0.0 ? c0 : a.op.initial_penalty;
        double cbar_inv = 1.0 / fmax(pen_c, 1.0);
        int nu = 0, inner_status = 0, state = D_INIT, final_status = 0;
        unsigned inner_total = 0, n_cost = 0, n_grad = 0, n_pass = 0;
        FlagBit f_start{fl, 1u << 7}, f_back{fl, 1u << 8}, f_trials{fl, 1u << 9}, f_end{fl, 1u << 10}, f_begin{fl, 1u << 11}, f_done{fl, 1u << 12}, f_fb{fl, 1u << 13};
        FlagBit running{fl, 1u << 14}, timed_out{fl, 1u << 15}, posted{fl, 1u << 16};
        f_start = true; running = true;

        unsigned q_pass = 0;
        FlagBit parked{fl, 1u << 5}, long_counted{fl, 1u << 6};
        int park_cls = POOL_LONG;
        if (resumed) {
            const double *pks = pk + 6 * N;
            pen_c = pks[0]; cbar_inv = 1.0 / fmax(pen_c, 1.0);
            eps_nu = pks[1]; dy_norm = pks[2]; f2_norm = pks[3]; dy_norm_plus = pks[4]; f2_norm_plus = pks[5]; last_fpr = pks[6]; last_cost = pks[7];
            nu = (int)pks[8]; inner_total = (unsigned)pks[9]; n_cost = (unsigned)pks[10]; n_grad = (unsigned)pks[11]; n_pass = (unsigned)pks[12];
            t_start = (long long)pks[13]; long_counted = pks[15] != 0.0; q_pass = n_pass;
        }
        if constexpr (TIMED) clk_dl = clk_deadline(clk_batch, a.tl_dur, t_start);

        for (;;) {
            bool lb_batch = false;
            if (fl & (f_back.bit | f_fb.bit)) {
                if (f_back) {
                    if (posted) { posted = false; if (lane == 0) ctl_store(ctl + CTL_CLAIM + wid, 0); }
                    lb_active = 0; lb_first = true;
                    NMPC2_LB_ZERO();
                    fbe_ok = false;
                    Lc *= 2.0; gamma /= 2.0;
                    sigma = (1.0 - GAMMA_L_COEFF) / (4.0 * gamma);
                    c_lip = GAMMA_L_COEFF / (2.0 * gamma);
                    Lpar[19] = 0.5 / gamma;
                    NMPC2_HALF_STEP(uv, uw);
                    lb_batch = true;
                }
                if (f_fb) {
                    f_fb = false;
                    tau = 0.0;
                    ld4<H2_COLS>(Cgk, tc, gv, gw);
                    NMPC2_HALF_STEP(uv, uw);
                    xv = yqv = hv; xw = yqw = hw; need_grad = true; state = D_FB;
                }
            }
            if (f_trials) {
                f_trials = false;
                const double th_ = h == 0 ? tau : tau / 2.0, omt = 1.0 - th_;
                xv = fma2(-th_, dv, fma2(-omt, rv, uv));
                xw = fma2(-th_, dw, fma2(-omt, rw, uw));
                const double t4_ = tau / 4.0, om4_ = 1.0 - t4_;
                yqv = fma2(-t4_, dv, fma2(-om4_, rv, uv));
                yqw = fma2(-t4_, dw, fma2(-om4_, rw, uw));
                need_grad = true; state = D_LS;
            }
            if (f_end) {
                f_end = false;
                iteration++;
                if (!(num_iter < max_inner)) f_done = true;
                else {
                    num_iter++;
                    if ((budget > 0u && inner_total + num_iter >= budget) || (TIMED && clk_reached(clk_dl))) { timed_out = true; f_done = true; }
                    else f_begin = true;
                }
            }
            if (f_begin) lb_batch = true;
            double gU = 0.0;
            D2 gs1 = d2s(0.0), gs2 = d2s(0.0), gy1 = d2s(0.0), gy2 = d2s(0.0);
            if (lb_batch) {
                rv = uv - hv; rw = uw - hw;
                if (f_begin && iteration >= 1 && !lb_first) {
                    D2 o1, o2, g1, g2;
                    ld4<H2_COLS>(Cos, tc, o1, o2);
                    ld4<H2_COLS>(Cog, tc, g1, g2);
                    gs1 = uv - o1; gs2 = uw - o2; gy1 = rv - g1; gy2 = rw - g2;
                }
                if (t < H2_NS - 1 && h == 0) {
                    st4<H2_NS>(Lnv, t, gs1, gs2); st4<H2_NS>(Lnv + 2 * H2_NS, t, gy1, gy2);
                    st4<H2_NS>(Lnv + 4 * H2_NS, t, rv, rw); st4<H2_NS>(Lnv + 6 * H2_NS, t, gv, gw);
                }
                const lds_double2 *X1 = (c16 < MAXMEM ? LS + 2 * H2_NS * c16 : (c16 == 11 ? Lnv + 4 * H2_NS : Lnv)) + 5 * q4;
                const lds_double2 *X2 = (c16 < MAXMEM ? LY + 2 * H2_NS * c16 : (c16 == 11 ? Lnv + 6 * H2_NS : Lnv + 2 * H2_NS)) + 5 * q4;
                const lds_double2 *Z1 = (c16 < MAXMEM ? Lnv + 2 * H2_NS : (c16 == 10 ? Lnv : Lnv + 4 * H2_NS)) + 5 * q4;
                const lds_double2 *Z2 = (c16 < MAXMEM ? Lnv + 4 * H2_NS : (c16 == 10 ? Lnv + 2 * H2_NS : Lnv + 4 * H2_NS)) + 5 * q4;
// ... 548 lines not shown
```

Before: 226,500.

## Repack LDS scalar and segment records for 16-byte paired loads

Reorders the scalar-parameter slots so that values used together sit in aligned pairs. Pads segment records from 5 to 6 doubles so every record starts on a 16-byte boundary. Scalar, segment and obstacle reads and writes then use 128-bit LDS pair accesses instead of individual 64-bit ones, which cuts LDS instruction count in the hot psi evaluation loops. In exchange, the segment area uses more LDS and the parameter-to-slot mapping becomes a packed lookup. Gathered segment loads with a stride of three slots may also change bank-conflict patterns.

```diff
diff --git a/mpc_trajectory_generator_amd/csrc/nmpc_eval.h b/mpc_trajectory_generator_amd/csrc/nmpc_eval.h
--- a/mpc_trajectory_generator_amd/csrc/nmpc_eval.h
+++ b/mpc_trajectory_generator_amd/csrc/nmpc_eval.h
@@ -62,8 +62,9 @@
     const bool in_r = t < N;
     const bool in = FULL ? true : in_r;
     const lds_double *sc = L + mp.sc;
-    const double x0 = sc[SC_X0], y0 = sc[SC_Y0], th0 = sc[SC_TH0];
-    const double xf = sc[SC_XF], yf = sc[SC_YF], thf = sc[SC_THF];
+    const dbl2 p0_ = lds_pair(sc + SC_X0), h0_ = lds_pair(sc + SC_TH0), pf_ = lds_pair(sc + SC_XF);
+    const double x0 = p0_.x, y0 = p0_.y, th0 = h0_.x;
+    const double xf = pf_.x, yf = pf_.y, thf = h0_.y;
 
     double ew_, ex_, ey_;
     auto prefix_ex = [lane](double v, double &excl) {
@@ -82,14 +83,16 @@
     const double half_c = 0.5 * c;
     NMPC_EVTICK(nmpc_pe, 0);
 
-    double acc = (sc[SC_RV] * zv) * zv;
-    acc = fma(sc[SC_RW] * zw, zw, acc);
+    const dbl2 r_ = lds_pair(sc + SC_RV);
+    double acc = (r_.x * zv) * zv;
+    acc = fma(r_.y * zw, zw, acc);
     const double dv = zv - vref;
     acc = fma(sc[SC_QV] * dv, dv, acc);
     {
         const double ddx = xp - xf, ddy = yp - yf, dth = th - thf;
-        acc = fma(sc[SC_Q], fma(ddx, ddx, ddy * ddy), acc);
-        acc = fma(sc[SC_QTH] * dth, dth, acc);
+        const dbl2 q_ = lds_pair(sc + SC_Q);
+        acc = fma(q_.x, fma(ddx, ddx, ddy * ddy), acc);
+        acc = fma(q_.y * dth, dth, acc);
     }
     double best = __builtin_inf();
     int bi = 0;
@@ -106,9 +109,7 @@
                 const lds_double *sg = L + mp.seg + SEG_STRIDE * i0c;
                 double wv[2 * WIN + 1][5];
 #pragma unroll
-                for (int j = 0; j <= 2 * WIN; ++j)
-#pragma unroll
-                    for (int f = 0; f < 5; ++f) wv[j][f] = sg[j * SEG_STRIDE + f];
+                for (int j = 0; j <= 2 * WIN; ++j) seg_read(sg + j * SEG_STRIDE, wv[j]);
 #pragma unroll
                 for (int j = 0; j <= 2 * WIN; ++j) {
                     const double px = xn - wv[j][0], py = yn - wv[j][1];
@@ -138,16 +139,12 @@
         double cur[2][5], nxt[2][5];
         double mout = __builtin_inf();
 #pragma unroll
-        for (int j = 0; j < 2; ++j)
-#pragma unroll
-            for (int f = 0; f < 5; ++f) cur[j][f] = sg[j * SEG_STRIDE + f];
+        for (int j = 0; j < 2; ++j) seg_read(sg + j * SEG_STRIDE, cur[j]);
 #pragma unroll SH::N > 0 ? (SH::N <= 20 ? 32 : 2) : 1
         for (int i = 0; i < nseg4; i += 2) {
             sg += 2 * SEG_STRIDE;
 #pragma unroll
-            for (int j = 0; j < 2; ++j)
-#pragma unroll
-                for (int f = 0; f < 5; ++f) nxt[j][f] = sg[j * SEG_STRIDE + f];
+            for (int j = 0; j < 2; ++j) seg_read(sg + j * SEG_STRIDE, nxt[j]);
             NMPC_SCHED_BARRIER();
             double d2[2];
 #pragma unroll
@@ -183,19 +180,22 @@
     }
     NMPC_EVTICK(nmpc_pe, 1);
     acc = fma(sc[SC_QCTE], best, acc);
-    const double vprev = evx ? evx->vprev : from_prev<P>(zv, lane, sc[SC_VINIT]);
-    const double wprev = evx ? evx->wprev : from_prev<P>(zw, lane, sc[SC_WINIT]);
+    double vprev, wprev;
+    if (evx) { vprev = evx->vprev; wprev = evx->wprev; }
+    else { const dbl2 u_ = lds_pair(sc + SC_VINIT); vprev = from_prev<P>(zv, lane, u_.x); wprev = from_prev<P>(zw, lane, u_.y); }
     double av = (zv - vprev) * inv_ts, aw = (zw - wprev) * inv_ts;
-    acc = fma(sc[SC_PA] * av, av, acc);
-    acc = fma(sc[SC_PW] * aw, aw, acc);
+    const dbl2 pa_ = lds_pair(sc + SC_PA);
+    acc = fma(pa_.x * av, av, acc);
+    acc = fma(pa_.y * aw, aw, acc);
     const double tv = fma(yv, cbar_inv, av), tw = fma(yw, cbar_inv, aw);
     double sv = tv - clampd(tv, k_amin, k_amax);
     double sw = tw - clampd(tw, -k_awmax, k_awmax);
     acc = fma(half_c, fma(sv, sv, sw * sw), acc);
     if (t == N - 1) {
         const double tx = xn - xf, ty = yn - yf, tth = thn - thf;
-        acc = fma(sc[SC_QN], fma(tx, tx, ty * ty), acc);
-        acc = fma(sc[SC_QTHN] * tth, tth, acc);
+        const dbl2 qn_ = lds_pair(sc + SC_QN);
+        acc = fma(qn_.x, fma(tx, tx, ty * ty), acc);
+        acc = fma(qn_.y * tth, tth, acc);
     }
     if (!in) { acc = 0.0; av = aw = sv = sw = 0.0; }
     av_out = av;
@@ -242,7 +242,8 @@
 #pragma unroll
                 for (int j = 0; j < 4; ++j) {
                     const lds_double *oj = ob + OBS_STRIDE * kk[j];
-                    od[4 * j] = oj[0]; od[4 * j + 1] = oj[1]; od[4 * j + 2] = oj[2]; od[4 * j + 3] = oc ? oj[3] : 0.0;
+                    const dbl2 c_ = lds_pair(oj), e_ = lds_pair(oj + 2);
+                    od[4 * j] = c_.x; od[4 * j + 1] = c_.y; od[4 * j + 2] = e_.x; od[4 * j + 3] = oc ? e_.y : 0.0;
                 }
                 NMPC_SCHED_BARRIER();
 #pragma unroll
@@ -259,8 +260,8 @@
             double od[16];
 #pragma unroll
             for (int j = 0; j < 4; ++j) {
-                od[4 * j] = ob[OBS_STRIDE * j]; od[4 * j + 1] = ob[OBS_STRIDE * j + 1]; od[4 * j + 2] = ob[OBS_STRIDE * j + 2];
-                od[4 * j + 3] = oc ? ob[OBS_STRIDE * j + 3] : 0.0;
+                const dbl2 c_ = lds_pair(ob + OBS_STRIDE * j), e_ = lds_pair(ob + OBS_STRIDE * j + 2);
+                od[4 * j] = c_.x; od[4 * j + 1] = c_.y; od[4 * j + 2] = e_.x; od[4 * j + 3] = oc ? e_.y : 0.0;
             }
             NMPC_SCHED_BARRIER();
 #pragma unroll
@@ -304,7 +305,8 @@
     }
     double gx = 0.0, gy = 0.0;
     if (want_grad) {
-        const lds_double *sg = L + mp.seg + SEG_STRIDE * bi;
+        double sg[5];
+        seg_read(L + mp.seg + SEG_STRIDE * bi, sg);
         const double px = xn - sg[0], py = yn - sg[1];
         const double dot = fma(px, sg[2], py * sg[3]);
         const double that = dot * sg[4];
@@ -322,7 +324,8 @@
             rem &= rem - 1;
             if (rem == 0ull) {
                 const lds_double *o0 = L + mp.obs + OBS_STRIDE * k0;
-                const double ax = o0[0], ay = o0[1], ar = o0[2];
+                const dbl2 a_ = lds_pair(o0);
+                const double ax = a_.x, ay = a_.y, ar = o0[2];
                 const double dx0 = xn - ax, dy0 = yn - ay;
                 const double h0 = fma(-dy0, dy0, fma(-dx0, dx0, ar));
                 const double f20 = group_sum<P>(in ? fmax(h0, 0.0) : 0.0, lane);
@@ -337,7 +340,8 @@
             const int k1 = __builtin_ctzll(rem);
             rem &= rem - 1;
             const lds_double *o0 = L + mp.obs + OBS_STRIDE * k0, *o1 = L + mp.obs + OBS_STRIDE * k1;
-            const double ax = o0[0], ay = o0[1], ar = o0[2], bx = o1[0], by = o1[1], br = o1[2];
+            const dbl2 a_ = lds_pair(o0), b_ = lds_pair(o1);
+            const double ax = a_.x, ay = a_.y, ar = o0[2], bx = b_.x, by = b_.y, br = o1[2];
             const double dx0 = xn - ax, dy0 = yn - ay, dx1 = xn - bx, dy1 = yn - by;
             const double h0 = fma(-dy0, dy0, fma(-dx0, dx0, ar)), h1 = fma(-dy1, dy1, fma(-dx1, dx1, br));
             const double f20 = group_sum<P>(in ? fmax(h0, 0.0) : 0.0, lane);
@@ -381,13 +385,14 @@
     NMPC_EVTICK(nmpc_pe, 3);
     if (!want_grad) return;
 
-    const double wq = t < N - 1 ? sc[SC_Q] : sc[SC_QN];
-    const double wth = t < N - 1 ? sc[SC_QTH] : sc[SC_QTHN];
+    const dbl2 w_ = lds_pair(sc + (t < N - 1 ? SC_Q : SC_QN));
+    const double wq = w_.x, wth = w_.y;
     gx = fma(2.0 * wq, xn - xf, gx);
     gy = fma(2.0 * wq, yn - yf, gy);
     double gt = (2.0 * wth) * (thn - thf);
-    double qa = fma(c, sv, (2.0 * sc[SC_PA]) * av);
-    double qw = fma(c, sw, (2.0 * sc[SC_PW]) * aw);
+    const dbl2 pb_ = lds_pair(sc + SC_PA);
+    double qa = fma(c, sv, (2.0 * pb_.x) * av);
+    double qw = fma(c, sw, (2.0 * pb_.y) * aw);
     if (!in) { gx = gy = gt = qa = qw = 0.0; }
     const double Sx = group_suffix<P>(gx, lane);
     const double Sy = group_suffix<P>(gy, lane);
@@ -398,10 +403,11 @@
     if (evx) { *evx->mine = dbl2{qa, qw}; const dbl2 n_ = *evx->next; qan = n_.x; qwn = n_.y; }
     else { qan = from_next<P>(qa, lane); qwn = from_next<P>(qw, lane); }
     const double dynv = fma(Sx, cs, Sy * sn);
-    double g1 = fma(2.0 * sc[SC_RV], zv, (2.0 * sc[SC_QV]) * dv);
+    const dbl2 rb_ = lds_pair(sc + SC_RV);
+    double g1 = fma(2.0 * rb_.x, zv, (2.0 * sc[SC_QV]) * dv);
     g1 = fma(inv_ts, qa - qan, g1);
     g1 = fma(ts, dynv, g1);
-    double g2 = (2.0 * sc[SC_RW]) * zw;
+    double g2 = (2.0 * rb_.y) * zw;
     g2 = fma(inv_ts, qw - qwn, g2);
     g2 = fma(ts, St, g2);
     gv = in ? g1 : 0.0;
diff --git a/mpc_trajectory_generator_amd/csrc/nmpc_layout.h b/mpc_trajectory_generator_amd/csrc/nmpc_layout.h
--- a/mpc_trajectory_generator_amd/csrc/nmpc_layout.h
+++ b/mpc_trajectory_generator_amd/csrc/nmpc_layout.h
@@ -1,4 +1,6 @@
 #pragma once
+
+#include "nmpc_lds_map.h"
 
 #ifndef NMPC_WIN
 #define NMPC_WIN 1
@@ -7,16 +9,6 @@
 namespace nmpc {
 
 constexpr int NZ = 20;
-constexpr int MAXMEM = 10;
-constexpr int NDYN_MAX = 3;
-constexpr int GRAM_LD = 11;
-constexpr int GRAM_NST = 20;
-constexpr int OBS_STRIDE = 4;
-constexpr int SEG_STRIDE = 5;
-constexpr int TEAM_WAVES = 4;
-constexpr int TEAM_REQ_DOUBLES = 3 * 24 * 2;
-constexpr int TEAM_AREA_DOUBLES = 3 * 24 * 2 + 8;
-constexpr int TEAM_CTL_INTS = 64;
 constexpr int NPOOLS = 2;
 enum { POOL_LONG = 0, POOL_COLD = 1 };
 
@@ -30,24 +22,6 @@
 constexpr int MAX_LINESEARCH_ITERATIONS = 10;
 constexpr double LBFGS_SY_EPSILON = 1e-10;
 constexpr double LBFGS_CBFGS_EPSILON = 1e-8;
-
-struct LdsMap {
-    int sc;
-    int cw;
-    int par;
-    int seg;
-    int obs;
-    int f2;
-    int dyn;
-    int dyn_stride;
-    int req;
-    int vec;
-    int rho;
-    int S, Y;
-    int nv;
-    int gsy, gyy;
-    int total;
-};
 
 struct KArgs {
     nmpc_problem pb;
@@ -91,12 +65,15 @@
     };
 };
 
-enum { SC_X0 = 0, SC_Y0, SC_TH0, SC_VINIT, SC_WINIT, SC_XF, SC_YF, SC_THF,
-       SC_Q, SC_QV, SC_QTH, SC_RV, SC_RW, SC_QN, SC_QTHN, SC_QCTE, SC_PA, SC_PW };
-
 typedef __attribute__((address_space(3))) double lds_double;
 typedef double dbl2 __attribute__((ext_vector_type(2)));
 typedef __attribute__((address_space(3))) dbl2 lds_double2;
+__device__ __forceinline__ dbl2 lds_pair(const lds_double *p) { return *(const lds_double2 *)p; }
+__device__ __forceinline__ void seg_read(const lds_double *sg, double (&f)[5])
+{
+    const dbl2 a = lds_pair(sg), d = lds_pair(sg + 2), i = lds_pair(sg + 4);
+    f[0] = a.x; f[1] = a.y; f[2] = d.x; f[3] = d.y; f[4] = i.x;
+}
 
 #ifdef NMPC_NO_SCHED_BARRIER
 #define NMPC_SCHED_BARRIER() do { } while (0)
@@ -128,51 +105,25 @@
 template <class SH> __device__ __forceinline__ int shape_nobs(const KArgs &a) { if constexpr (SH::NOBS >= 0) return SH::NOBS; else return a.pb.nobs; }
 template <class SH> __device__ __forceinline__ int shape_ndyn(const KArgs &a) { if constexpr (SH::NDYN >= 0) return SH::NDYN; else return a.pb.ndyn; }
 
-__host__ __device__ constexpr LdsMap lds_layout(int N, int nobs, int ndyn, int P)
-{
-    LdsMap mp{};
-    int o = 0;
-    mp.sc = o;  o += 20;
-    mp.cw = o;  o += CW_NCOEF;
-    mp.par = o; o += 24;
-    mp.seg = o; o += SEG_STRIDE * (N + 5);
-    mp.obs = o; o += OBS_STRIDE * (nobs + 4);
-    const int points = P == 64 ? 1 : 3;
-    mp.f2 = o;  o += P == 20 ? 0 : points * (nobs + ndyn + 1);
-    mp.rho = o; o += MAXMEM;
-    const int cols = P == 20 ? 24 : P;
-    mp.dyn_stride = P == 64 ? ((N + 1) & ~1) : (P == 20 ? 24 : P);
-    mp.dyn = o; o += NDYN_MAX * 6 * mp.dyn_stride;
-    o = (o + 1) & ~1;
-    mp.req = o; o += P == 20 ? TEAM_REQ_DOUBLES : 0;
-    mp.vec = o; o += P == 64 ? 0 : 7 * 2 * cols;
-    if (P == 20) { mp.f2 = mp.vec; if (7 * 2 * cols < points * (nobs + ndyn + 1)) o = mp.vec + points * (nobs + ndyn + 1); }
-    o = (o + 1) & ~1;
-    mp.gsy = o; o += P == 20 ? MAXMEM * GRAM_LD : 0;
-    mp.gyy = o; o += P == 20 ? MAXMEM * GRAM_LD : 0;
-    const int ring = P == 20 ? GRAM_NST + 1 : N;
-    mp.S = o;   o += 2 * ring * MAXMEM;
-    mp.Y = o;   o += 2 * ring * MAXMEM;
-    mp.nv = o;  o += P == 20 ? 4 * 2 * GRAM_NST : 0;
-    mp.total = (o + 1) & ~1;
-    if (P == 20 && mp.total < 3 * TEAM_WAVES * TEAM_AREA_DOUBLES) mp.total = 3 * TEAM_WAVES * TEAM_AREA_DOUBLES;
-    return mp;
-}
 template <class SH, int P> __device__ __forceinline__ LdsMap the_map(const KArgs &a)
 {
     if constexpr (SH::N > 0 && SH::NOBS >= 0 && SH::NDYN >= 0) return lds_layout(SH::N, SH::NOBS, SH::NDYN, P);
     else return a.map;
 }
 
+static_assert(LDS_CW_SLOTS == CW_NCOEF, "the slice's coefficient table");
+__device__ __forceinline__ void sc_write(lds_double *sc, const double *p, int lane)
+{
+    constexpr unsigned long long lo = sc_slot_word(0), hi = sc_slot_word(10);
+    if (lane < 20 && lane != 8 && lane != 9) sc[(int)(((lane < 10 ? lo : hi) >> (5 * (lane < 10 ? lane : lane - 10))) & 31)] = p[lane];
+}
 template <int P, class SH = ShapeAny>
 __device__ __forceinline__ void prepare_instance(const KArgs &a, lds_double *L, const double *p, int t,
                                                  double &vref, DynStage &dyn)
 {
     const int N = shape_N<SH>(a), nobs = shape_nobs<SH>(a), ndyn = shape_ndyn<SH>(a);
     const LdsMap mp = the_map<SH, P>(a);
-    if (t < 8) L[mp.sc + t] = p[t];
-    if (t >= 8 && t < 18) L[mp.sc + t] = p[t + 2];
-    if (t == 18 || t == 19) L[mp.sc + t] = p[t - 15];
+    sc_write(L + mp.sc, p, t);
     if (t < CW_NCOEF) L[mp.cw + t] = CW_COEF_DEV[t];
     NMPC_WAVE_SYNC();
     vref = t < N ? p[NZ + t] : 0.0;
@@ -180,10 +131,9 @@
     for (int k = t; k < ((nobs + 4) & ~3); k += P) {
         const bool real = k < nobs;
         const double r = real ? ps[3 * k + 2] : 0.0;
-        L[mp.obs + OBS_STRIDE * k] = real ? ps[3 * k] : 0.0;
-        L[mp.obs + OBS_STRIDE * k + 1] = real ? ps[3 * k + 1] : 0.0;
-        L[mp.obs + OBS_STRIDE * k + 2] = r * r;
-        L[mp.obs + OBS_STRIDE * k + 3] = r > 0.0 ? r : -1e30;
+        lds_double2 *ob = (lds_double2 *)(L + mp.obs + OBS_STRIDE * k);
+        ob[0] = dbl2{real ? ps[3 * k] : 0.0, real ? ps[3 * k + 1] : 0.0};
+        ob[1] = dbl2{r * r, r > 0.0 ? r : -1e30};
     }
     const double *pd = ps + 3 * nobs;
     {
@@ -219,12 +169,10 @@
         const double ax = pr[3 * i], ay = pr[3 * i + 1];
         const double bx = pr[3 * i + 3], by = pr[3 * i + 4];
         const double dx = bx - ax, dy = by - ay;
-        lds_double *sg = L + mp.seg + SEG_STRIDE * t;
-        sg[0] = ax;
-        sg[1] = ay;
-        sg[2] = dx;
-        sg[3] = dy;
-        sg[4] = 1.0 / (fma(dx, dx, dy * dy) + 1e-16);
+        lds_double2 *sg = (lds_double2 *)(L + mp.seg + SEG_STRIDE * t);
+        sg[0] = dbl2{ax, ay};
+        sg[1] = dbl2{dx, dy};
+        sg[2] = dbl2{1.0 / (fma(dx, dx, dy * dy) + 1e-16), 0.0};
     }
     NMPC_WAVE_SYNC();
 }
diff --git a/mpc_trajectory_generator_amd/csrc/nmpc_lds_map.h b/mpc_trajectory_generator_amd/csrc/nmpc_lds_map.h
--- /dev/null
+++ b/mpc_trajectory_generator_amd/csrc/nmpc_lds_map.h
@@ -0,0 +1,94 @@
+#pragma once
+
+#ifdef __HIPCC__
+#define NMPC_HD __host__ __device__
+#else
+#define NMPC_HD
+#endif
+
+namespace nmpc {
+
+constexpr int MAXMEM = 10;
+constexpr int NDYN_MAX = 3;
+constexpr int GRAM_LD = 11;
+constexpr int GRAM_NST = 20;
+constexpr int LDS_CW_SLOTS = 10;
+constexpr int OBS_STRIDE = 4;
+constexpr int SEG_STRIDE = 6;
+constexpr int SEG_STRIDE_PACKED = 5, SC_DOUBLES = 20;
+static_assert(SEG_STRIDE % 2 == 0 && (SEG_STRIDE / 2) % 2 == 1 && OBS_STRIDE % 2 == 0, "records: whole 16-byte slots; gathered ones an odd number of them");
+
+constexpr int TEAM_WAVES = 4;
+constexpr int TEAM_REQ_DOUBLES = 3 * 24 * 2;
+constexpr int TEAM_AREA_DOUBLES = 3 * 24 * 2 + 8;
+constexpr int TEAM_CTL_INTS = 64;
+
+enum { SC_X0 = 0, SC_Y0, SC_TH0, SC_THF, SC_XF, SC_YF, SC_VINIT, SC_WINIT,
+       SC_RV, SC_RW, SC_Q, SC_QTH, SC_QV, SC_QCTE, SC_PA, SC_PW, SC_QN, SC_QTHN, SC_USED };
+static_assert(SC_USED <= SC_DOUBLES && SC_X0 % 2 == 0 && SC_TH0 % 2 == 0 && SC_XF % 2 == 0 && SC_VINIT % 2 == 0 && SC_RV % 2 == 0 &&
+              SC_Q % 2 == 0 && SC_QV % 2 == 0 && SC_PA % 2 == 0 && SC_QN % 2 == 0, "pairs start on even slots");
+NMPC_HD constexpr int sc_slot_of_param(int i)
+{
+    constexpr signed char slot[20] = {SC_X0, SC_Y0, SC_TH0, SC_VINIT, SC_WINIT, SC_XF, SC_YF, SC_THF, -1, -1,
+                                      SC_Q, SC_QV, SC_QTH, SC_RV, SC_RW, SC_QN, SC_QTHN, SC_QCTE, SC_PA, SC_PW};
+    return slot[i];
+}
+NMPC_HD constexpr unsigned long long sc_slot_word(int first)
+{
+    unsigned long long w = 0;
+    for (int i = 0; i < 10; ++i) w |= (unsigned long long)(sc_slot_of_param(first + i) & 31) << (5 * i);
+    return w;
+}
+
+struct LdsMap {
+    int sc;
+    int cw;
+    int par;
+    int seg;
+    int obs;
+    int f2;
+    int dyn;
+    int dyn_stride;
+    int req;
+    int vec;
+    int rho;
+    int S, Y;
+    int nv;
+    int gsy, gyy;
+    int total;
+};
+
+NMPC_HD constexpr LdsMap lds_layout(int N, int nobs, int ndyn, int P, int seg_stride = SEG_STRIDE)
+{
+    LdsMap mp{};
+    int o = 0;
+    mp.sc = o;  o += SC_DOUBLES;
+    mp.cw = o;  o += LDS_CW_SLOTS;
+    mp.par = o; o += 24;
+    mp.seg = o; o += seg_stride * (N + 5);
+    mp.obs = o; o += OBS_STRIDE * (nobs + 4);
+    const int points = P == 64 ? 1 : 3;
+    mp.f2 = o;  o += P == 20 ? 0 : points * (nobs + ndyn + 1);
+    mp.rho = o; o += MAXMEM;
+    const int cols = P == 20 ? 24 : P;
+    mp.dyn_stride = P == 64 ? ((N + 1) & ~1) : (P == 20 ? 24 : P);
+    mp.dyn = o; o += NDYN_MAX * 6 * mp.dyn_stride;
+    o = (o + 1) & ~1;
+    mp.req = o; o += P == 20 ? TEAM_REQ_DOUBLES : 0;
+    mp.vec = o; o += P == 64 ? 0 : 7 * 2 * cols;
+    if (P == 20) { mp.f2 = mp.vec; if (7 * 2 * cols < points * (nobs + ndyn + 1)) o = mp.vec + points * (nobs + ndyn + 1); }
+    o = (o + 1) & ~1;
+    mp.gsy = o; o += P == 20 ? MAXMEM * GRAM_LD : 0;
+    mp.gyy = o; o += P == 20 ? MAXMEM * GRAM_LD : 0;
+    const int ring = P == 20 ? GRAM_NST + 1 : N;
+    mp.S = o;   o += 2 * ring * MAXMEM;
+    mp.Y = o;   o += 2 * ring * MAXMEM;
+    mp.nv = o;  o += P == 20 ? 4 * 2 * GRAM_NST : 0;
+    mp.total = (o + 1) & ~1;
+    if (P == 20 && mp.total < 3 * TEAM_WAVES * TEAM_AREA_DOUBLES) mp.total = 3 * TEAM_WAVES * TEAM_AREA_DOUBLES;
+    return mp;
+}
+static_assert((SC_DOUBLES + LDS_CW_SLOTS + 24) % 2 == 0, "the segment table starts 16-byte aligned");
+static_assert(8 * 8 * lds_layout(20, 10, 3, 20).total + 2 * 4 * TEAM_CTL_INTS <= 160 * 1024, "two workgroups of the hybrid kernel per CU");
+
+}
diff --git a/mpc_trajectory_generator_amd/csrc/nmpc_solve_hyb.h b/mpc_trajectory_generator_amd/csrc/nmpc_solve_hyb.h
--- a/mpc_trajectory_generator_amd/csrc/nmpc_solve_hyb.h
+++ b/mpc_trajectory_generator_amd/csrc/nmpc_solve_hyb.h
@@ -242,7 +242,7 @@
     lds_double2 *zwX = Lz + (t < ZS ? h * ZS + t : 3 * ZS + (t - ZS));
     lds_double2 *zwY = Lz + (t < ZS ? 2 * ZS + t : 3 * ZS + (t - ZS));
     const lds_double2 *zrd = Lz + q * ZS + te;
-    const lds_double2 *zpv = te == 0 ? (const lds_double2 *)(L + mp.sc + 18) : (lane < 60 ? zrd - 1 : zrd);
+    const lds_double2 *zpv = te == 0 ? (const lds_double2 *)(L + mp.sc + SC_VINIT) : (lane < 60 ? zrd - 1 : zrd);
     lds_double2 *zmine = Lz + (lane < 60 ? q * ZS + te : 3 * ZS + (lane - 60));
     const lds_double2 *znext = Lz + opaque_i(lane < 60 ? q * ZS + te + 1 : 3 * ZS + (lane - 60) + 1);
     const lds_double2 *zgr = Lz + (t < 20 ? t : 20);
diff --git a/mpc_trajectory_generator_amd/csrc/nmpc_solve_hyb2.h b/mpc_trajectory_generator_amd/csrc/nmpc_solve_hyb2.h
--- a/mpc_trajectory_generator_amd/csrc/nmpc_solve_hyb2.h
+++ b/mpc_trajectory_generator_amd/csrc/nmpc_solve_hyb2.h
@@ -66,7 +66,7 @@
 {
     LdsMap2 mp{};
     int o = 0;
-    mp.sc = o;  o += 20;
+    mp.sc = o;  o += SC_DOUBLES;
     mp.cw = o;  o += CW_NCOEF;
     mp.par = o; o += 20;
     mp.seg = o; o += SEG_STRIDE * (N + 5);
@@ -91,6 +91,7 @@
     mp.total = (o + 1) & ~1;
     return mp;
 }
+static_assert(8 * lds_layout2(40, 10, 3).total <= 40 * 1024, "a CU holds four slices of the two-stage kernel's headline shape");
 template <class SH> __device__ __forceinline__ LdsMap2 the_map2(const KArgs &a)
 {
     if constexpr (SH::N > 0 && SH::NOBS >= 0 && SH::NDYN >= 0) return lds_layout2(SH::N, SH::NOBS, SH::NDYN);
@@ -101,8 +102,7 @@
 __device__ __forceinline__ void prepare_instance2(const KArgs &a, lds_double *L, const LdsMap2 &mp, const double *p, int lane)
 {
     const int N = shape_N<SH>(a), nobs = shape_nobs<SH>(a), ndyn = shape_ndyn<SH>(a);
-    if (lane < 8) L[mp.sc + lane] = p[lane];
-    if (lane >= 8 && lane < 18) L[mp.sc + lane] = p[lane + 2];
+    sc_write(L + mp.sc, p, lane);
     if (lane < CW_NCOEF) L[mp.cw + lane] = CW_COEF_DEV[lane];
     NMPC_WAVE_SYNC();
     if (lane < 48) L[mp.vr + lane] = lane < N ? p[NZ + lane] : 0.0;
@@ -110,10 +110,9 @@
     for (int k = lane; k < ((nobs + 3) & ~3); k += 64) {
         const bool real = k < nobs;
         const double r = real ? ps[3 * k + 2] : 0.0;
-        L[mp.obs + OBS_STRIDE * k] = real ? ps[3 * k] : 0.0;
-        L[mp.obs + OBS_STRIDE * k + 1] = real ? ps[3 * k + 1] : 0.0;
-        L[mp.obs + OBS_STRIDE * k + 2] = r * r;
-        L[mp.obs + OBS_STRIDE * k + 3] = r > 0.0 ? r : -1e30;
+        lds_double2 *ob = (lds_double2 *)(L + mp.obs + OBS_STRIDE * k);
+        ob[0] = dbl2{real ? ps[3 * k] : 0.0, real ? ps[3 * k + 1] : 0.0};
+        ob[1] = dbl2{r * r, r > 0.0 ? r : -1e30};
     }
     const double *pd = ps + 3 * nobs;
     if (lane < 48) {
@@ -144,12 +143,10 @@
         const double ax = pr[3 * i], ay = pr[3 * i + 1];
         const double bx = pr[3 * i + 3], by = pr[3 * i + 4];
         const double dx = bx - ax, dy = by - ay;
-        lds_double *sg = L + mp.seg + SEG_STRIDE * lane;
-        sg[0] = ax;
-        sg[1] = ay;
-        sg[2] = dx;
-        sg[3] = dy;
-        sg[4] = 1.0 / (fma(dx, dx, dy * dy) + 1e-16);
+        lds_double2 *sg = (lds_double2 *)(L + mp.seg + SEG_STRIDE * lane);
+        sg[0] = dbl2{ax, ay};
+        sg[1] = dbl2{dx, dy};
+        sg[2] = dbl2{1.0 / (fma(dx, dx, dy * dy) + 1e-16), 0.0};
     }
     NMPC_WAVE_SYNC();
 }
@@ -177,8 +174,9 @@
     const bool ina = FULL ? true : ra, inb = FULL ? true : rb;
     const lds_double *sc = L + mp.sc;
     const lds_double *cw = (const lds_double *)(L + mp.cw);
-    const double x0 = sc[SC_X0], y0 = sc[SC_Y0], th0 = sc[SC_TH0];
-    const double xf = sc[SC_XF], yf = sc[SC_YF], thf = sc[SC_THF];
+    const dbl2 p0_ = lds_pair(sc + SC_X0), h0_ = lds_pair(sc + SC_TH0), pf_ = lds_pair(sc + SC_XF);
+    const double x0 = p0_.x, y0 = p0_.y, th0 = h0_.x;
+    const double xf = pf_.x, yf = pf_.y, thf = h0_.y;
     D2 vref;
     { const dbl2 v = ((const lds_double2 *)(L + mp.vr))[te]; vref = D2{v.x, v.y}; }
 
@@ -193,17 +191,20 @@
     const D2 yp = prev2(yn, lane, y0);
     const double half_c = 0.5 * c;
 
-    D2 acc = (sc[SC_RV] * zv) * zv;
-    acc = fma2(sc[SC_RW] * zw, zw, acc);
+    const dbl2 r_ = lds_pair(sc + SC_RV);
+    D2 acc = (r_.x * zv) * zv;
+    acc = fma2(r_.y * zw, zw, acc);
     const D2 dv = zv - vref;
     acc = fma2(sc[SC_QV] * dv, dv, acc);
     {
         const D2 ddx = xp - d2s(xf), ddy = yp - d2s(yf), dth = th - d2s(thf);
-        acc = fma2(sc[SC_Q], fma2(ddx, ddx, ddy * ddy), acc);
-        acc = fma2(sc[SC_QTH] * dth, dth, acc);
-    }
-    const D2 vprev = prev2(zv, lane, sc[SC_VINIT]);
-    const D2 wprev = prev2(zw, lane, sc[SC_WINIT]);
+        const dbl2 q_ = lds_pair(sc + SC_Q);
+        acc = fma2(q_.x, fma2(ddx, ddx, ddy * ddy), acc);
+        acc = fma2(q_.y * dth, dth, acc);
+    }
+    const dbl2 u_ = lds_pair(sc + SC_VINIT);
+    const D2 vprev = prev2(zv, lane, u_.x);
+    const D2 wprev = prev2(zw, lane, u_.y);
     D2 best = d2s(__builtin_inf());
     int bia = 0, bib = 0;
     bool full_scan = true;
@@ -222,8 +223,9 @@
                     double bst = __builtin_inf();                                                          \
                     int bi_ = 0;                                                                           \
                     _Pragma("unroll") for (int j = 0; j <= 2 * WIN; ++j) {                                 \
-                        const double s0 = sg[j * SEG_STRIDE], s1 = sg[j * SEG_STRIDE + 1], s2 = sg[j * SEG_STRIDE + 2], \
-                                     s3 = sg[j * SEG_STRIDE + 3], s4 = sg[j * SEG_STRIDE + 4];             \
+                        double sf[5];                                                                      \
+                        seg_read(sg + j * SEG_STRIDE, sf);                                                 \
+                        const double s0 = sf[0], s1 = sf[1], s2 = sf[2], s3 = sf[3], s4 = sf[4];           \
                         const double px = xn.S_ - s0, py = yn.S_ - s1;                                     \
                         const double dot = fma(s2, px, s3 * py);                                           \
                         const double tst = fmin(fmax(s4 * dot, 0.0), 1.0);                                 \
@@ -255,16 +257,12 @@
         double cur[2][5], nxt[2][5];
         D2 mout = d2s(__builtin_inf());
 #pragma unroll
-        for (int j = 0; j < 2; ++j)
-#pragma unroll
-            for (int f = 0; f < 5; ++f) cur[j][f] = sg[j * SEG_STRIDE + f];
+        for (int j = 0; j < 2; ++j) seg_read(sg + j * SEG_STRIDE, cur[j]);
 #pragma unroll SH::N > 0 ? 4 : 1
         for (int i = 0; i < nseg4; i += 2) {
             sg += 2 * SEG_STRIDE;
 #pragma unroll
-            for (int j = 0; j < 2; ++j)
-#pragma unroll
-                for (int f = 0; f < 5; ++f) nxt[j][f] = sg[j * SEG_STRIDE + f];
+            for (int j = 0; j < 2; ++j) seg_read(sg + j * SEG_STRIDE, nxt[j]);
             NMPC_SCHED_BARRIER();
             D2 d2v[2];
 #pragma unroll
@@ -301,21 +299,24 @@
     }
     acc = fma2(sc[SC_QCTE], best, acc);
     D2 av = inv_ts * (zv - vprev), aw = inv_ts * (zw - wprev);
-    acc = fma2(sc[SC_PA] * av, av, acc);
-    acc = fma2(sc[SC_PW] * aw, aw, acc);
+    const dbl2 pa_ = lds_pair(sc + SC_PA);
+    acc = fma2(pa_.x * av, av, acc);
+    acc = fma2(pa_.y * aw, aw, acc);
     const D2 tv = fma2(cbar_inv, yv, av), tw = fma2(cbar_inv, yw, aw);
     D2 sv = tv - clamp2(tv, a.pb.amin, a.pb.amax);
     D2 sw = tw - clamp2(tw, -a.pb.awmax, a.pb.awmax);
     acc = fma2(half_c, fma2(sv, sv, sw * sw), acc);
     if (sa_ == N - 1) {
         const double tx = xn.a - xf, ty = yn.a - yf, tth = thn.a - thf;
-        acc.a = fma(sc[SC_QN], fma(tx, tx, ty * ty), acc.a);
-        acc.a = fma(sc[SC_QTHN] * tth, tth, acc.a);
+        const dbl2 qn_ = lds_pair(sc + SC_QN);
+        acc.a = fma(qn_.x, fma(tx, tx, ty * ty), acc.a);
+        acc.a = fma(qn_.y * tth, tth, acc.a);
     }
     if (sb_ == N - 1) {
         const double tx = xn.b - xf, ty = yn.b - yf, tth = thn.b - thf;
-        acc.b = fma(sc[SC_QN], fma(tx, tx, ty * ty), acc.b);
-        acc.b = fma(sc[SC_QTHN] * tth, tth, acc.b);
+        const dbl2 qn_ = lds_pair(sc + SC_QN);
+        acc.b = fma(qn_.x, fma(tx, tx, ty * ty), acc.b);
+        acc.b = fma(qn_.y * tth, tth, acc.b);
     }
     if (!ina) { acc.a = 0.0; av.a = aw.a = sv.a = sw.a = 0.0; }
     if (!inb) { acc.b = 0.0; av.b = aw.b = sv.b = sw.b = 0.0; }
@@ -346,8 +347,8 @@
             double od[16];
 #pragma unroll
             for (int j = 0; j < 4; ++j) {
-                od[4 * j] = ob[OBS_STRIDE * j]; od[4 * j + 1] = ob[OBS_STRIDE * j + 1]; od[4 * j + 2] = ob[OBS_STRIDE * j + 2];
-                od[4 * j + 3] = oc ? ob[OBS_STRIDE * j + 3] : 0.0;
+                const dbl2 c_ = lds_pair(ob + OBS_STRIDE * j), e_ = lds_pair(ob + OBS_STRIDE * j + 2);
+                od[4 * j] = c_.x; od[4 * j + 1] = c_.y; od[4 * j + 2] = e_.x; od[4 * j + 3] = oc ? e_.y : 0.0;
             }
             NMPC_SCHED_BARRIER();
 #pragma unroll
@@ -390,7 +391,8 @@
         const double two_q = 2.0 * sc[SC_QCTE];
 #define NMPC_CTE_ADJ(S_, BI_)                                                              \
         do {                                                                               \
-            const lds_double *sg = L + mp.seg + SEG_STRIDE * (BI_);                        \
+            double sg[5];                                                                  \
+            seg_read(L + mp.seg + SEG_STRIDE * (BI_), sg);                                 \
             const double px = xn.S_ - sg[0], py = yn.S_ - sg[1];                           \
             const double dot = fma(px, sg[2], py * sg[3]);                                 \
             const double that = dot * sg[4];                                               \
@@ -410,7 +412,8 @@
             const int k0 = __builtin_ctzll(rem);
             rem &= rem - 1;
             const lds_double *o0 = L + mp.obs + OBS_STRIDE * k0;
-            const double ax = o0[0], ay = o0[1], ar = o0[2];
+            const dbl2 a_ = lds_pair(o0);
+            const double ax = a_.x, ay = a_.y, ar = o0[2];
             const D2 dx0 = xn - d2s(ax), dy0 = yn - d2s(ay);
             const D2 h0 = fma2(-dy0, dy0, fma2(-dx0, dx0, d2s(ar)));
             const double f20 = gsum2(D2{ina ? fmax(h0.a, 0.0) : 0.0, inb ? fmax(h0.b, 0.0) : 0.0}, lane);
@@ -449,13 +452,15 @@
     pen_out = pen;
     if (!want_grad) return;
 
-    const D2 wq = D2{sa_ < N - 1 ? sc[SC_Q] : sc[SC_QN], sb_ < N - 1 ? sc[SC_Q] : sc[SC_QN]};
-    const D2 wth = D2{sa_ < N - 1 ? sc[SC_QTH] : sc[SC_QTHN], sb_ < N - 1 ? sc[SC_QTH] : sc[SC_QTHN]};
+    const dbl2 wa_ = lds_pair(sc + (sa_ < N - 1 ? SC_Q : SC_QN)), wb_ = lds_pair(sc + (sb_ < N - 1 ? SC_Q : SC_QN));
+    const D2 wq = D2{wa_.x, wb_.x};
+    const D2 wth = D2{wa_.y, wb_.y};
     gx = fma2(2.0 * wq, xn - d2s(xf), gx);
     gy = fma2(2.0 * wq, yn - d2s(yf), gy);
     D2 gt = (2.0 * wth) * (thn - d2s(thf));
-    D2 qa = fma2(c, sv, (2.0 * sc[SC_PA]) * av);
-    D2 qw = fma2(c, sw, (2.0 * sc[SC_PW]) * aw);
+    const dbl2 pb_ = lds_pair(sc + SC_PA);
+    D2 qa = fma2(c, sv, (2.0 * pb_.x) * av);
+    D2 qw = fma2(c, sw, (2.0 * pb_.y) * aw);
     if (!ina) { gx.a = gy.a = gt.a = qa.a = qw.a = 0.0; }
     if (!inb) { gx.b = gy.b = gt.b = qa.b = qw.b = 0.0; }
     const D2 Sx = gsuffix2(gx, lane);
@@ -470,10 +475,11 @@
     const D2 St = gsuffix2(stin, lane);
     const D2 qan = next2(qa, lane), qwn = next2(qw, lane);
     const D2 dynv = fma2(Sx, cs, Sy * sn);
-    D2 g1 = fma2(2.0 * sc[SC_RV], zv, (2.0 * sc[SC_QV]) * dv);
+    const dbl2 rb_ = lds_pair(sc + SC_RV);
+    D2 g1 = fma2(2.0 * rb_.x, zv, (2.0 * sc[SC_QV]) * dv);
     g1 = fma2(inv_ts, qa - qan, g1);
     g1 = fma2(ts, dynv, g1);
-    D2 g2 = (2.0 * sc[SC_RW]) * zw;
+    D2 g2 = (2.0 * rb_.y) * zw;
     g2 = fma2(inv_ts, qw - qwn, g2);
     g2 = fma2(ts, St, g2);
     gv = D2{ina ? g1.a : 0.0, inb ? g1.b : 0.0};
```

New measurement: 225,100. Within noise of the previous version (-0.6%).
